# kevslinger/DTQN

Measured on AMD Instinct MI355X. Metric: env-steps/sec + TD-updates/sec, DiscreteCarFlag-v0 ctx=50 b=32, 1/2/4/8 GPU, higher is better.
Workload: dtype f32; 1 GPU; DiscreteCarFlag-v0 shapes (BASELINE config 1): ctx=50, d_model=64, 8 heads, 2 layers, obs 3 f32, 3 actions, batch 32 per GPU, history 50, device replay 2500 x 200 steps; global_batch=32, parallelism=dp1, sampler=device

## Files before the change

### dtqn_amd/_binding.py

```python
from __future__ import annotations

import ctypes
import os
import re
from typing import Dict, List, Tuple

REPO = os.path.dirname(os.path.dirname(os.path.abspath(__file__)))
HEADER = os.path.join(REPO, "include", "dtqn_hip.h")

_SCALARS = {
    "int32_t": ctypes.c_int32, "uint32_t": ctypes.c_uint32, "float": ctypes.c_float, "int": ctypes.c_int,
}


def _strip_comments(src: str) -> str:
    src = re.sub(r"/\*.*?\*/", "", src, flags=re.S)
    return re.sub(r"//[^\n]*", "", src)


def parse_structs(header_path: str = HEADER) -> Dict[str, List[Tuple[str, object]]]:
    src = _strip_comments(open(header_path).read())
    out: Dict[str, List[Tuple[str, object]]] = {}
    for m in re.finditer(r"typedef\s+struct\s+(\w+)\s*\{(.*?)\}\s*(\w+)\s*;", src, flags=re.S):
        name, body = m.group(3), m.group(2)
        fields: List[Tuple[str, object]] = []
        for decl in body.split(";"):
            decl = " ".join(decl.split())
            if not decl:
                continue
            if "*" in decl:
                for nm in decl.split("*")[-1].split(","):
                    fields.append((nm.strip(), ctypes.c_void_p))
                continue
            toks = decl.split(" ", 1)
            ctype = _SCALARS[toks[0]]
            for nm in toks[1].split(","):
                fields.append((nm.strip(), ctype))
        out[name] = fields
    return out


def parse_defines(header_path: str = HEADER) -> Dict[str, int]:
    src = _strip_comments(open(header_path).read())
    return {m.group(1): int(m.group(2)) for m in re.finditer(r"#define\s+(DTQN_\w+)\s+(-?\d+)\s*$", src, flags=re.M)}


def parse_functions(header_path: str = HEADER) -> List[str]:
    src = _strip_comments(open(header_path).read())
    src = re.sub(r"typedef\s+struct.*?\}\s*\w+\s*;", "", src, flags=re.S)
    return re.findall(r"\b(dtqn_\w+)\s*\(", src)


_STRUCTS = parse_structs()
DEFINES = parse_defines()
FUNCTIONS = sorted(set(parse_functions()))


def _make(name: str):
    return type(name, (ctypes.Structure,), {"_fields_": _STRUCTS[name]})


DtqnNet = _make("DtqnNet")
DtqnWJob = _make("DtqnWJob")
DtqnReplay = _make("DtqnReplay")
DtqnReplayRecord = _make("DtqnReplayRecord")
DtqnTd = _make("DtqnTd")


def load_library(path: str) -> ctypes.CDLL:
    lib = ctypes.CDLL(path)
    missing = [f for f in FUNCTIONS if not hasattr(lib, f)]
    if missing:
        raise OSError(f"{path} does not export {missing} (declared in include/dtqn_hip.h)")
    vp, i32, u32 = ctypes.c_void_p, ctypes.c_int, ctypes.c_uint32
    P = ctypes.POINTER
    protos = {
        "dtqn_net_init": [P(DtqnNet)],
        "dtqn_net_wjobs": [P(DtqnNet), P(DtqnWJob)],
        "dtqn_net_fill_frozen": [P(DtqnNet), vp],
        "dtqn_lds_bytes_forward": [P(DtqnNet), i32],
        "dtqn_lds_bytes_backward": [P(DtqnNet)],
        "dtqn_replay_apply": [P(DtqnReplay), vp, vp, i32, vp],
        "dtqn_replay_sample": [P(DtqnReplay), i32, i32, i32, i32, u32, vp, vp, vp, vp],
        "dtqn_replay_sample_at": [P(DtqnReplay), i32, i32, i32, i32, u32, i32, vp, vp, vp, vp],
        "dtqn_replay_push": [P(DtqnReplay), vp, vp, i32, vp],
        "dtqn_td_prefers_tiled": [P(DtqnNet), i32],
        "dtqn_net_tiled_twin": [P(DtqnNet), P(DtqnNet)],
        "dtqn_replay_gather_bag": [P(DtqnReplay), vp, vp, vp, i32, i32, u32, vp, vp, vp, vp],
        "dtqn_actor_forward": [P(DtqnNet), vp, vp, vp, i32, vp, vp, vp, i32, u32, u32, vp],
        "dtqn_actor_forward_batch": [P(DtqnNet), vp, vp, vp, i32, i32, vp, vp, vp, i32, u32, u32, vp],
        "dtqn_actor_greedy_batch": [P(DtqnNet), vp, vp, vp, i32, i32, vp, vp, vp, vp, i32, u32, u32, vp],
        "dtqn_debug_last_actor_live": [],
        "dtqn_forward_tiled_strided": [P(DtqnNet), vp, vp, vp, i32, i32, i32, vp, vp, vp],
        "dtqn_forward_bag": [P(DtqnNet), vp, vp, vp, vp, vp, i32, i32, vp, vp, i32, u32, u32, vp],
        "dtqn_forward": [P(DtqnNet), vp, vp, vp, i32, i32, vp, vp],
        "dtqn_forward_workspace_floats": [P(DtqnNet), i32],
        "dtqn_forward_tiled": [P(DtqnNet), vp, vp, vp, i32, i32, vp, vp, vp],
        "dtqn_td_row_split": [P(DtqnNet), i32],
        "dtqn_td_latency_mode": [P(DtqnNet), i32],
        "dtqn_td_wgrad_is_direct": [P(DtqnNet), i32],
        "dtqn_td_wgrad_splits": [P(DtqnNet), i32],
        "dtqn_td_wpack_floats": [P(DtqnNet)],
        "dtqn_td_wpack": [P(DtqnNet), P(DtqnTd), vp],
        "dtqn_td_wgrad_is_fused": [P(DtqnNet), P(DtqnTd)],
        "dtqn_td_norm_partials": [P(DtqnNet)],
        "dtqn_td_xch_floats": [P(DtqnNet), i32],
        "dtqn_td_xch_flags": [P(DtqnNet), i32],
        "dtqn_td_forward": [P(DtqnNet), P(DtqnReplay), P(DtqnTd), vp],
        "dtqn_td_forward_part": [P(DtqnNet), P(DtqnReplay), P(DtqnTd), i32, i32, i32, i32, vp],
        "dtqn_td_fwd_slices4_ok": [P(DtqnNet)],
        "dtqn_td_backward": [P(DtqnNet), P(DtqnReplay), P(DtqnTd), vp],
        "dtqn_td_backward_ahead": [P(DtqnNet), P(DtqnReplay), P(DtqnTd), P(DtqnTd), i32, vp],
        "dtqn_td_wgrad": [P(DtqnNet), P(DtqnTd), vp],
        "dtqn_td_reduce": [P(DtqnNet), P(DtqnTd), vp],
        "dtqn_td_gradnorm": [P(DtqnNet), P(DtqnTd), vp],
        "dtqn_td_clip_adam": [P(DtqnNet), P(DtqnTd), vp],
        "dtqn_img_prep_floats": [P(DtqnNet)],
        "dtqn_img_act_floats": [P(DtqnNet), i32],
        "dtqn_img_gact_floats": [P(DtqnNet), i32],
        "dtqn_img_wpart_floats": [P(DtqnNet)],
        "dtqn_img_prep": [P(DtqnNet), vp, vp, vp],
        "dtqn_img_encode": [P(DtqnNet), vp, vp, vp, vp, i32, vp, vp, vp, vp, vp, vp],
        "dtqn_img_backward": [P(DtqnNet), vp, vp, vp, vp, i32, vp, vp, vp, vp, vp, vp, vp],
        "dtqn_img_td_lists": [P(DtqnNet), P(DtqnReplay), P(DtqnTd), vp, vp, vp, vp, vp, vp, vp],
        "dtqn_forward_tiled_pre": [P(DtqnNet), vp, vp, vp, i32, i32, vp, vp, i32, u32, u32, vp],
        "dtqn_img_actor_stage_bytes": [P(DtqnNet), i32],
        "dtqn_img_actor_workspace_floats": [P(DtqnNet), i32],
        "dtqn_img_actor_forward_batch": [P(DtqnNet), vp, vp, i32, vp, vp, vp, i32, vp, vp, vp, i32, u32, u32, vp],
        "dtqn_img_actor_greedy_batch": [P(DtqnNet), vp, vp, i32, vp, vp, vp, i32, vp, vp, vp, vp, i32, u32, u32, vp],
        "dtqn_debug_last_img_actor_tokens": [],
        "dtqn_grad_workspace_floats": [P(DtqnNet), i32, i32],
        "dtqn_forward_train": [P(DtqnNet), vp, vp, vp, vp, vp, i32, i32, vp, vp, vp],
        "dtqn_backward_dq": [P(DtqnNet), vp, vp, vp, vp, vp, i32, i32, vp, vp, vp, vp, vp],
        "dtqn_forward_train_drop": [P(DtqnNet), vp, vp, vp, vp, vp, i32, i32, vp, vp, u32, i32, vp],
        "dtqn_backward_dq_drop": [P(DtqnNet), vp, vp, vp, vp, vp, i32, i32, vp, vp, vp, vp, u32, i32, vp],
        "dtqn_attn_weights": [P(DtqnNet), vp, i32, i32, vp, vp, vp],
        "dtqn_xch_publish": [vp, i32, vp],
        "dtqn_td_xreduce": [P(DtqnNet), P(DtqnTd), vp, vp, i32, i32, vp, vp, vp, vp],
        "dtqn_td_update": [P(DtqnNet), P(DtqnReplay), P(DtqnTd), vp],
        "dtqn_td_update_pipelined": [P(DtqnNet), P(DtqnReplay), P(DtqnTd), P(DtqnTd), i32, i32, vp],
        "dtqn_td_gradients_pipelined": [P(DtqnNet), P(DtqnReplay), P(DtqnTd), P(DtqnTd), i32, i32, vp],
        "dtqn_target_sync": [P(DtqnNet), vp, vp, vp],
        "dtqn_debug_set_profile_buffer": [vp],
        "dtqn_debug_last_packed_blocks": [],
        "dtqn_abi_version": [],
        "dtqn_build_info": [],
    }
    for name, argtypes in protos.items():
        fn = getattr(lib, name)
        fn.argtypes = argtypes
        fn.restype = ctypes.c_char_p if name == "dtqn_build_info" else (
            ctypes.c_longlong if name in ("dtqn_img_act_floats", "dtqn_img_gact_floats", "dtqn_img_wpart_floats",
                                                    "dtqn_grad_workspace_floats", "dtqn_img_actor_stage_bytes",
                                                    "dtqn_img_actor_workspace_floats") else ctypes.c_int)
    assert set(protos) == set(FUNCTIONS), sorted(set(protos) ^ set(FUNCTIONS))
    if lib.dtqn_abi_version() != DEFINES["DTQN_ABI_VERSION"]:
        raise OSError(f"{path}: ABI version {lib.dtqn_abi_version()} != header {DEFINES['DTQN_ABI_VERSION']}")
    return lib


GATES = {"res": DEFINES["DTQN_GATE_RES"], "gru": DEFINES["DTQN_GATE_GRU"]}
POS = {"learned": DEFINES["DTQN_POS_LEARNED"], "sin": DEFINES["DTQN_POS_SIN"], "none": DEFINES["DTQN_POS_NONE"]}


def make_net(lib, *, obs_dim, num_actions, embed_per_obs_dim=8, action_dim=0, inner_embed_size=64, num_heads=8,
             num_layers=2, history_len=50, gate="res", identity=False, pos="learned", discrete=False,
             vocab_sizes=0, dropout=0.0, bag_size=0, image=None) -> DtqnNet:
    net = DtqnNet()
    net.obs_dim, net.num_actions, net.embed_per_obs, net.action_dim = obs_dim, num_actions, embed_per_obs_dim, action_dim
    net.d_model, net.num_heads, net.num_layers, net.ctx_len = inner_embed_size, num_heads, num_layers, history_len
    if gate not in GATES:
        raise ValueError("Gate must be one of `gru`, `res`")
    net.gate, net.identity, net.pos = GATES[gate], int(bool(identity)), POS[str(pos)]
    net.discrete, net.vocab = int(bool(discrete)), int(vocab_sizes or 0)
    net.dropout = float(dropout)
    net.bag_size = int(bag_size)
    if image is not None:
        net.img_c, net.img_h, net.img_w = (int(v) for v in image)
        net.obs_dim = net.img_c * net.img_h * net.img_w
    rc = lib.dtqn_net_init(ctypes.byref(net))
    if rc != 0:
        raise NotImplementedError(
            f"dtqn_net_init rc={rc}: this DTQN variant/shape is outside the gfx950 kernels' coverage "
            f"(D={inner_embed_size}, H={num_heads}, L={history_len}, gate={gate}, dropout={dropout}, bag_size={bag_size}); see DESIGN.md")
    return net


def param_table(net: DtqnNet, width: int = 0) -> Dict[str, Tuple[int, Tuple[int, ...]]]:
    D, L, A, a = (width or net.d_model), net.ctx_len, net.num_actions, net.action_dim
    tab: Dict[str, Tuple[int, Tuple[int, ...]]] = {}
    if a > 0:
        tab["action_embedding.embedding.0.weight"] = (net.off_act_emb, (A, a))
    if net.img_c > 0:
        chans = [(net.img_c, 64), (64, 64), (64, 64), (64, 128), (128, 128)]
        offs = [(net.off_cw0, net.off_cb0), (net.off_cw1, net.off_cb1), (net.off_cw2, net.off_cb2), (net.off_cw3, net.off_cb3), (net.off_cw4, net.off_cb4)]
        for i, ((ci, co), (ow, ob)) in enumerate(zip(chans, offs)):
            tab[f"obs_embedding.observation_embedding.{2 * i}.weight"] = (ow, (co, ci, 3, 3))
            tab[f"obs_embedding.observation_embedding.{2 * i}.bias"] = (ob, (co,))
        tab["obs_embedding.observation_embedding.11.weight"] = (net.off_obs_w, (D - a, net.ke))
        tab["obs_embedding.observation_embedding.11.bias"] = (net.off_obs_b, (D - a,))
    elif net.discrete:
        tab["obs_embedding.observation_embedding.0.weight"] = (net.off_obs_tab, (net.vocab, net.embed_per_obs))
        tab["obs_embedding.observation_embedding.2.weight"] = (net.off_obs_w, (D - a, net.ke))
        tab["obs_embedding.observation_embedding.2.bias"] = (net.off_obs_b, (D - a,))
    else:
        tab["obs_embedding.observation_embedding.weight"] = (net.off_obs_w, (D - a, net.ke))
        tab["obs_embedding.observation_embedding.bias"] = (net.off_obs_b, (D - a,))
    tab["position_embedding.position_encoding"] = (net.off_pos, (1, L, D))
    gate_names = [("w_r.weight", net.go_w_r, (D, D)), ("u_r.weight", net.go_u_r, (D, D)),
                  ("w_z.weight", net.go_w_z, (D, D)), ("w_z.bias", net.go_b_z, (D,)),
                  ("u_z.weight", net.go_u_z, (D, D)), ("w_g.weight", net.go_w_g, (D, D)),
                  ("u_g.weight", net.go_u_g, (D, D))]
    for l in range(net.num_layers):
        base = net.off_layer0 + l * net.layer_stride
        pre = f"transformer_layers.{l}."
        tab[pre + "layernorm1.weight"] = (base + net.lo_ln1_w, (D,))
        tab[pre + "layernorm1.bias"] = (base + net.lo_ln1_b, (D,))
        tab[pre + "layernorm2.weight"] = (base + net.lo_ln2_w, (D,))
        tab[pre + "layernorm2.bias"] = (base + net.lo_ln2_b, (D,))
        tab[pre + "attention.in_proj_weight"] = (base + net.lo_in_w, (3 * D, D))
        tab[pre + "attention.in_proj_bias"] = (base + net.lo_in_b, (3 * D,))
        tab[pre + "attention.out_proj.weight"] = (base + net.lo_out_w, (D, D))
        tab[pre + "attention.out_proj.bias"] = (base + net.lo_out_b, (D,))
        tab[pre + "ffn.0.weight"] = (base + net.lo_f1_w, (4 * D, D))
        tab[pre + "ffn.0.bias"] = (base + net.lo_f1_b, (4 * D,))
        tab[pre + "ffn.2.weight"] = (base + net.lo_f2_w, (D, 4 * D))
        tab[pre + "ffn.2.bias"] = (base + net.lo_f2_b, (D,))
        if net.gate == GATES["gru"]:
            for gname, goff in (("attn_gate", net.off_gate_attn), ("mlp_gate", net.off_gate_mlp)):
                for nm, off, shp in gate_names:
                    tab[pre + f"{gname}.{nm}"] = (goff + off, shp)
    if net.bag_size > 0:
        tab["bag_attention.in_proj_weight"] = (net.off_bag_in_w, (3 * D, D))
        tab["bag_attention.in_proj_bias"] = (net.off_bag_in_b, (3 * D,))
        tab["bag_attention.out_proj.weight"] = (net.off_bag_out_w, (D, D))
        tab["bag_attention.out_proj.bias"] = (net.off_bag_out_b, (D,))
    tab["ffn.0.weight"] = (net.off_head1_w, (D, 2 * D if net.bag_size > 0 else D))
    tab["ffn.0.bias"] = (net.off_head1_b, (D,))
    tab["ffn.2.weight"] = (net.off_head2_w, (A, D))
    tab["ffn.2.bias"] = (net.off_head2_b, (A,))
    return tab


def ws_lite(net: DtqnNet) -> bool:
    return (not net.tiled) and net.d_model == 64 and (net.head_dim == 32 or (net.d_real > 0 and net.head_dim in (8, 16)))


def _grids(net: DtqnNet, key: str, real_shape, padded_shape):
    H, Hp = net.heads_real or net.num_heads, net.num_heads
    hd, hdp = net.hd_real or net.head_dim, net.head_dim
    if key.endswith("attention.in_proj_weight") or key.endswith("attention.in_proj_bias"):
        return (3, H, hd) + tuple(real_shape[1:]), (3, Hp, hdp) + tuple(padded_shape[1:])
    if key.endswith("attention.out_proj.weight"):
        return (real_shape[0], H, hd), (padded_shape[0], Hp, hdp)
    return tuple(real_shape), tuple(padded_shape)


def unpad_param(net: DtqnNet, key: str, padded, real_shape):
    if not net.d_real or tuple(padded.shape) == tuple(real_shape):
        return padded
    rg, pg = _grids(net, key, real_shape, padded.shape)
    return padded.reshape(pg)[tuple(slice(0, r) for r in rg)].reshape(tuple(real_shape))


def pad_param(net: DtqnNet, key: str, real, padded_shape):
    if not net.d_real or tuple(real.shape) == tuple(padded_shape):
        return real
    import numpy as _np
    out = _np.zeros(padded_shape, dtype=real.dtype) if isinstance(real, _np.ndarray) else real.new_zeros(tuple(padded_shape))
    rg, pg = _grids(net, key, real.shape, padded_shape)
    out.reshape(pg)[tuple(slice(0, r) for r in rg)] = real.reshape(rg)
    return out
```

### dtqn_amd/csrc/dtqn_api.cpp

```cpp
#include <hip/hip_runtime.h>

#include <cstdlib>

#include "dtqn_hip.h"
#include "dtqn_limits.h"

extern "C" const char* dtqn_build_info(void) {
#ifdef DTQN_BUILD_INFO
    return DTQN_BUILD_INFO;
#else
    return "dtqn_hip (unstamped build)";
#endif
}

static void* g_profile_buffer = nullptr;
extern "C" int dtqn_debug_set_profile_buffer(void* dev_buffer) {
    g_profile_buffer = dev_buffer;
    return DTQN_OK;
}
extern "C" void* dtqn_debug_profile_buffer(void) { return g_profile_buffer; }

static int policy_cus() {
    int dev = 0, n = 0;
    if (hipGetDevice(&dev) != hipSuccess || hipDeviceGetAttribute(&n, hipDeviceAttributeMultiprocessorCount, dev) != hipSuccess || n <= 0) return 256;
    return n;
}
extern "C" int dtqn_td_row_split(const DtqnNet* net, int batch) {
    if (!net || batch < 1) return 1;
    const int cus = policy_cus();
    const char* e = getenv("DTQN_ROW_SPLIT");
    if (e != nullptr && e[0] == '0') return 1;
    const bool covered = !net->tiled && net->lp == 64 && !net->identity &&
                         (net->d_model == 64 || (net->d_model == 128 && net->gate == DTQN_GATE_RES));
    if (!covered) return 1;
    if (e != nullptr && e[0] == '1') return 2;
    if (e != nullptr && e[0] == '4') return 4;
    if (3 * batch * 2 <= cus) return 4;
    if (net->d_model == 64) {
        if (batch * 4 <= cus) return 4;
        if (batch * 2 <= cus) return 2;
    }
    return 1;
}
extern "C" int dtqn_td_latency_mode(const DtqnNet* net, int batch) {
    if (dtqn_td_row_split(net, batch) < 2) return 0;
    const char* e = getenv("DTQN_ROW_SPLIT");
    if (e != nullptr && (e[0] == '1' || e[0] == '4')) return 1;
    return 3 * batch * 2 <= policy_cus() ? 1 : 0;
}
extern "C" int dtqn_td_prefers_tiled(const DtqnNet* net, int batch) {
    if (!net || batch < 1 || net->tiled) return 0;
    if (dtqn_ws_lite(net->tiled, net->d_model, net->head_dim, net->d_real))
        return dtqn_td_row_split(net, batch) == 4 && dtqn_td_latency_mode(net, batch) ? 0 : 1;
    const bool covered = net->d_model == 128 && net->gate == DTQN_GATE_RES && !net->identity && net->lp == 64 && net->dropout == 0.f &&
                         net->bag_size == 0;
    if (!covered) return 0;
    const char* e = getenv("DTQN_TRAIN_TILED");
    if (e != nullptr) return atoi(e) != 0 ? 1 : 0;
    return dtqn_td_row_split(net, batch) == 1 ? 1 : 0;
}
extern "C" int dtqn_td_xch_floats(const DtqnNet* net, int batch) {
    if (!net || batch < 1) return 0;
    return 3 * batch * net->num_layers * (3 * net->lp / 4) * 2 * net->d_model;
}
extern "C" int dtqn_td_xch_flags(const DtqnNet* net, int batch) {
    if (!net || batch < 1) return 0;
    return 3 * batch * net->num_layers * 6 + 16;
}

extern "C" int dtqn_td_update(const DtqnNet* net, const DtqnReplay* rp, const DtqnTd* td, void* stream) {
    int rc;
    if ((rc = dtqn_td_forward(net, rp, td, stream)) != DTQN_OK) return rc;
    if ((rc = dtqn_td_backward(net, rp, td, stream)) != DTQN_OK) return rc;
    if ((rc = dtqn_td_wgrad(net, td, stream)) != DTQN_OK) return rc;
    if ((rc = dtqn_td_reduce(net, td, stream)) != DTQN_OK) return rc;
    return dtqn_td_clip_adam(net, td, stream);
}

extern "C" int dtqn_td_gradients_pipelined(const DtqnNet* net, const DtqnReplay* rp, const DtqnTd* td, const DtqnTd* td_next, int have_target,
                                           int draw_step, void* stream) {
    int rc;
    if (draw_step < 0) return DTQN_ERR_ARG;
    if ((rc = dtqn_td_forward_part(net, rp, td, 0, 2, 4, draw_step, stream)) != DTQN_OK) return rc;
    if (!have_target && (rc = dtqn_td_forward_part(net, rp, td, 2, 1, 4, draw_step, stream)) != DTQN_OK) return rc;
    rc = td_next != nullptr ? dtqn_td_backward_ahead(net, rp, td, td_next, draw_step + 1, stream) : dtqn_td_backward(net, rp, td, stream);
    if (rc != DTQN_OK) return rc;
    if ((rc = dtqn_td_wgrad(net, td, stream)) != DTQN_OK) return rc;
    return dtqn_td_reduce(net, td, stream);
}
extern "C" int dtqn_td_update_pipelined(const DtqnNet* net, const DtqnReplay* rp, const DtqnTd* td, const DtqnTd* td_next, int have_target,
                                        int draw_step, void* stream) {
    const int rc = dtqn_td_gradients_pipelined(net, rp, td, td_next, have_target, draw_step, stream);
    return rc != DTQN_OK ? rc : dtqn_td_clip_adam(net, td, stream);
}

namespace dtqn {
int forward_infer(const DtqnNet* net, const float* theta, const float* obs, const uint8_t* actions, int batch, int n,
                  float* q_out, float* q_last_host, void* stream, float* xch, int32_t* xflags, const int32_t* last_rows, int in_rows,
                  uint32_t drop_seed, uint32_t drop_step, int train_mode);
int tiled_forward_actor(const DtqnNet* net, const float* theta, const float* obs, const uint8_t* actions, int batch, int n, int in_rows,
                        float* q_out, float* workspace, int train_mode, uint32_t drop_seed, uint32_t drop_step, hipStream_t stream, const int32_t* lens = nullptr);
int actor_compact(const DtqnNet* net, const void* ctx_host, void* ctx_dev, int n_envs, int n_max, hipStream_t stream);
int actor_greedy_rows(const int32_t* lens, const float* q, float* q_last, int32_t* action, int n_envs, int n_max, int A, hipStream_t stream);
void set_last_actor_live(int live);
}
extern "C" int dtqn_forward_tiled_strided(const DtqnNet* net, const float* theta, const float* obs, const uint8_t* actions,
                                          int batch, int n, int in_rows, float* q_out, float* workspace, void* stream);

extern "C" int dtqn_replay_push(const DtqnReplay* rp, const DtqnReplayRecord* recs_host, const float* obs_host, int n,
                                void* stream) {
    if (!rp || n < 0) return DTQN_ERR_ARG;
    if (n == 0) return DTQN_OK;
    if (!recs_host || !obs_host) return DTQN_ERR_ARG;
    return dtqn_replay_apply(rp, recs_host, obs_host, n, stream);
}

extern "C" int dtqn_actor_forward(const DtqnNet* net, const float* theta, const void* ctx_host, void* ctx_dev, int n,
                                  float* q_dev, float* q_last_host, float* workspace, int train_mode, uint32_t dropout_seed,
                                  uint32_t dropout_step, void* stream) {
    if (!net || !theta || !ctx_host || !ctx_dev || !q_dev || !q_last_host) return DTQN_ERR_ARG;
    if (n < 1 || n > net->ctx_len) return DTQN_ERR_ARG;
    hipStream_t s = (hipStream_t)stream;
    const size_t obs_bytes = sizeof(float) * (size_t)net->ctx_len * net->obs_dim;
    if (hipMemcpyAsync(ctx_dev, ctx_host, obs_bytes + (size_t)net->ctx_len, hipMemcpyHostToDevice, s) != hipSuccess) return DTQN_ERR_LAUNCH;
    const float* obs = static_cast<const float*>(ctx_dev);
    const uint8_t* actions = static_cast<const uint8_t*>(ctx_dev) + obs_bytes;
    if (!net->tiled) {
        const bool split = workspace != nullptr && n > net->lp / 2 && dtqn_td_row_split(net, 1) >= 2;
        float* xch = split ? workspace : nullptr;
        int32_t* xflags = split ? reinterpret_cast<int32_t*>(workspace + dtqn_td_xch_floats(net, 1)) : nullptr;
        return dtqn::forward_infer(net, theta, obs, actions, 1, n, q_dev, q_last_host, stream, xch, xflags, nullptr, 0, dropout_seed, dropout_step, train_mode);
    }
    const int rc = dtqn::tiled_forward_actor(net, theta, obs, actions, 1, n, n, q_dev, workspace, train_mode, dropout_seed, dropout_step, s);
    if (rc != DTQN_OK) return rc;
    if (hipMemcpyAsync(q_last_host, q_dev + (size_t)(n - 1) * net->num_actions, sizeof(float) * net->num_actions,
                       hipMemcpyDeviceToHost, s) != hipSuccess)
        return DTQN_ERR_LAUNCH;
    return DTQN_OK;
}

struct ActorBlock {
    const float* obs;
    const uint8_t* actions;
    const int32_t* lens;
};
static ActorBlock actor_block(const DtqnNet* net, void* base, int n_envs) {
    const size_t obs_bytes = sizeof(float) * (size_t)n_envs * net->ctx_len * net->obs_dim;
    const size_t act_bytes = (((size_t)n_envs * net->ctx_len) + 3) & ~(size_t)3;
    const uint8_t* p = static_cast<const uint8_t*>(base);
    return ActorBlock{static_cast<const float*>(base), p + obs_bytes, reinterpret_cast<const int32_t*>(p + obs_bytes + act_bytes)};
}
static int actor_batch_forward(const DtqnNet* net, const float* theta, const ActorBlock& b, int batch, int ws_envs, int n_max, float* q_dev,
                               float* q_last_host, float* workspace, int train_mode, uint32_t dropout_seed, uint32_t dropout_step,
                               void* stream) {
    const int L = net->ctx_len;
    if (net->tiled)
        return dtqn::tiled_forward_actor(net, theta, b.obs, b.actions, batch, n_max, L, q_dev, workspace, train_mode, dropout_seed,
                                         dropout_step, (hipStream_t)stream, b.lens);
    const bool split = workspace != nullptr && n_max > net->lp / 2 && dtqn_td_row_split(net, batch) >= 2;
    float* xch = split ? workspace : nullptr;
    int32_t* xflags = split ? reinterpret_cast<int32_t*>(workspace + dtqn_td_xch_floats(net, ws_envs)) : nullptr;
    return dtqn::forward_infer(net, theta, b.obs, b.actions, batch, n_max, q_dev, q_last_host, stream, xch, xflags, b.lens, L, dropout_seed,
                               dropout_step, train_mode);
}

extern "C" int dtqn_actor_forward_batch(const DtqnNet* net, const float* theta, const void* ctx_host, void* ctx_dev, int n_envs,
                                        int n_max, float* q_dev, float* q_last_host, float* workspace, int train_mode,
                                        uint32_t dropout_seed, uint32_t dropout_step, void* stream) {
    if (!net || !theta || !ctx_host || !ctx_dev || !q_dev || !q_last_host || n_envs < 1) return DTQN_ERR_ARG;
    if (n_max < 1 || n_max > net->ctx_len) return DTQN_ERR_ARG;
    hipStream_t s = (hipStream_t)stream;
    const int L = net->ctx_len;
    const size_t obs_bytes = sizeof(float) * (size_t)n_envs * L * net->obs_dim;
    const size_t act_bytes = (((size_t)n_envs * L) + 3) & ~(size_t)3;
    const size_t total = obs_bytes + act_bytes + sizeof(int32_t) * (size_t)n_envs;
    const int32_t* lens_h = reinterpret_cast<const int32_t*>(static_cast<const uint8_t*>(ctx_host) + obs_bytes + act_bytes);
    for (int i = 0; i < n_envs; ++i)
        if (lens_h[i] < 1 || lens_h[i] > n_max) return DTQN_ERR_ARG;
    if (hipMemcpyAsync(ctx_dev, ctx_host, total, hipMemcpyHostToDevice, s) != hipSuccess) return DTQN_ERR_LAUNCH;
    const ActorBlock b = actor_block(net, ctx_dev, n_envs);
    const int rc = actor_batch_forward(net, theta, b, n_envs, n_envs, n_max, q_dev, q_last_host, workspace, train_mode, dropout_seed,
                                       dropout_step, stream);
    if (rc != DTQN_OK || !net->tiled) return rc;
    for (int i = 0; i < n_envs; ++i)
        if (hipMemcpyAsync(q_last_host + (size_t)i * net->num_actions, q_dev + ((size_t)i * n_max + (lens_h[i] - 1)) * net->num_actions,
                           sizeof(float) * net->num_actions, hipMemcpyDeviceToHost, s) != hipSuccess)
            return DTQN_ERR_LAUNCH;
    return DTQN_OK;
}

extern "C" int dtqn_actor_greedy_batch(const DtqnNet* net, const float* theta, const void* ctx_host, void* ctx_dev, int n_envs,
                                       int n_max, float* q_dev, float* q_last_host, int32_t* action_host, float* workspace,
                                       int train_mode, uint32_t dropout_seed, uint32_t dropout_step, void* stream) {
    if (!net || !theta || !ctx_host || !ctx_dev || !q_dev || !q_last_host || !action_host || n_envs < 1) return DTQN_ERR_ARG;
    if (n_max < 0 || n_max > net->ctx_len) return DTQN_ERR_ARG;
    const ActorBlock h = actor_block(net, const_cast<void*>(ctx_host), n_envs);
    int live = 0;
    for (int i = 0; i < n_envs; ++i) {
        if (h.lens[i] < 0 || h.lens[i] > n_max) return DTQN_ERR_ARG;
        live += h.lens[i] > 0 ? 1 : 0;
    }
    dtqn::set_last_actor_live(live);
    if (live == 0) {
        for (int i = 0; i < n_envs; ++i) action_host[i] = -1;
        return DTQN_OK;
    }
    hipStream_t s = (hipStream_t)stream;
    int rc;
    if ((rc = dtqn::actor_compact(net, ctx_host, ctx_dev, n_envs, n_max, s)) != DTQN_OK) return rc;
    const ActorBlock b = actor_block(net, ctx_dev, n_envs);
    if ((rc = actor_batch_forward(net, theta, b, live, n_envs, n_max, q_dev, nullptr, workspace, train_mode, dropout_seed, dropout_step,
                                  stream)) != DTQN_OK)
        return rc;
    return dtqn::actor_greedy_rows(h.lens, q_dev, q_last_host, action_host, n_envs, n_max, net->num_actions, s);
}

extern "C" int dtqn_forward_train(const DtqnNet* net, const float* theta, const float* obs, const uint8_t* actions, const float* bag_obs,
                                  const uint8_t* bag_actions, int batch, int n, float* q_out, float* workspace, void* stream) {
    return dtqn_forward_train_drop(net, theta, obs, actions, bag_obs, bag_actions, batch, n, q_out, workspace, 0u, -1, stream);
}
extern "C" int dtqn_backward_dq(const DtqnNet* net, const float* theta, const float* obs, const uint8_t* actions, const float* bag_obs,
                                const uint8_t* bag_actions, int batch, int n, const float* dq, float* workspace, float* grad, float* dobs,
                                void* stream) {
    return dtqn_backward_dq_drop(net, theta, obs, actions, bag_obs, bag_actions, batch, n, dq, workspace, grad, dobs, 0u, -1, stream);
}
```

### dtqn_amd/csrc/dtqn_optim.hip

```cpp
#include <cstdlib>

#include "dtqn_device.hpp"

namespace dtqn {

constexpr int kOptThreads = 256;
constexpr int kOptVec = 4;
constexpr int kOptBlockElems = kOptThreads * kOptVec;

struct ReduceArgs {
    DtqnNet net;
    const float* gsplit;
    const float* small;
    const float* grd;
    float* grad;
    float* norm_partial;
    int32_t* step_counter;
    int batch, n_split;
    int n_parts;
};

__device__ __forceinline__ float block_sum(float v, float* red, int tid) {
    for (int m = 32; m >= 1; m >>= 1) v += __shfl_xor(v, m);
    if ((tid & 63) == 0) red[tid >> 6] = v;
    __syncthreads();
    float s = 0.f;
    for (int w = 0; w < kOptThreads / 64; ++w) s += red[w];
    __syncthreads();
    return s;
}

__global__ __launch_bounds__(kOptThreads) void dtqn_reduce_kernel(ReduceArgs a) {
    __shared__ float red[kOptThreads / 64];
    const DtqnNet& net = a.net;
    const int tid = (int)threadIdx.x;
    const int p0 = ((int)blockIdx.x * kOptThreads + tid) * kOptVec;
    if (blockIdx.x == 0 && tid == 0) a.step_counter[0] = a.step_counter[1];
    if (blockIdx.x == 0)
        for (int i = (int)gridDim.x + tid; i < a.n_parts; i += kOptThreads) a.norm_partial[i] = 0.f;
    float v[kOptVec] = {0.f, 0.f, 0.f, 0.f};
    if (p0 < net.n_trainable) {
        for (int s = 0; s < a.n_split; ++s) {
            const float4 x = ld4(a.gsplit + (size_t)s * net.n_trainable + p0);
            v[0] += x.x; v[1] += x.y; v[2] += x.z; v[3] += x.w;
        }
        st4(a.grad + p0, make_float4(v[0], v[1], v[2], v[3]));
    }
    const float ss = block_sum((v[0] * v[0] + v[1] * v[1]) + (v[2] * v[2] + v[3] * v[3]), red, tid);
    if (tid == 0) a.norm_partial[blockIdx.x] = ss;
}

struct NormArgs {
    const float* grad;
    float* norm_partial;
    int n, n_parts;
};
__global__ __launch_bounds__(kOptThreads) void dtqn_gradnorm_kernel(NormArgs a) {
    __shared__ float red[kOptThreads / 64];
    const int tid = (int)threadIdx.x;
    const int p0 = ((int)blockIdx.x * kOptThreads + tid) * kOptVec;
    if (blockIdx.x == 0)
        for (int i = (int)gridDim.x + tid; i < a.n_parts; i += kOptThreads) a.norm_partial[i] = 0.f;
    float ss = 0.f;
    if (p0 < a.n) {
        const float4 g = ld4(a.grad + p0);
        ss = (g.x * g.x + g.y * g.y) + (g.z * g.z + g.w * g.w);
    }
    ss = block_sum(ss, red, tid);
    if (tid == 0) a.norm_partial[blockIdx.x] = ss;
}

struct PublishArgs {
    int32_t* flag;
    int32_t gen;
};
__global__ void dtqn_xch_publish_kernel(PublishArgs a) {
    if (threadIdx.x == 0 && blockIdx.x == 0) DTQN_SYSTEM_STORE(a.flag, a.gen);
}
struct XreduceArgs {
    const float* const* peer_grad;
    int32_t* const* peer_flag;
    float* gsum;
    float* norm_partial;
    int32_t* status;
    int n, n_parts, world;
    int32_t gen;
    long long timeout_ticks;
    int32_t* own_flag;
};
__global__ __launch_bounds__(kOptThreads) void dtqn_xreduce_kernel(XreduceArgs a) {
    __shared__ float red[kOptThreads / 64];
    const int tid = (int)threadIdx.x;
    if (blockIdx.x == 0)
        for (int i = (int)gridDim.x + tid; i < a.n_parts; i += kOptThreads) a.norm_partial[i] = 0.f;
    if (a.own_flag != nullptr && blockIdx.x == 0 && tid == 0) DTQN_SYSTEM_STORE(a.own_flag, a.gen);
    if (tid < a.world) {
        const int32_t* f = a.peer_flag[tid];
        const long long t0 = wall_clock64();
        while ((int32_t)(DTQN_SYSTEM_LOAD(f) - a.gen) < 0) {
            if (wall_clock64() - t0 > a.timeout_ticks || DTQN_SYSTEM_LOAD(a.status) != 0) {
                DTQN_SYSTEM_STORE(a.status, (int32_t)1);
                break;
            }
            DTQN_SPIN_PAUSE();
        }
    }
    __syncthreads();
    const int p0 = ((int)blockIdx.x * kOptThreads + tid) * kOptVec;
    float v[kOptVec] = {0.f, 0.f, 0.f, 0.f};
    if (p0 < a.n) {
        for (int r = 0; r < a.world; ++r) {
            const int32_t* g = reinterpret_cast<const int32_t*>(a.peer_grad[r] + p0);
#pragma unroll
            for (int c = 0; c < kOptVec; ++c) v[c] += __int_as_float(DTQN_SYSTEM_LOAD(g + c));
        }
        st4(a.gsum + p0, make_float4(v[0], v[1], v[2], v[3]));
    }
    const float ss = block_sum((v[0] * v[0] + v[1] * v[1]) + (v[2] * v[2] + v[3] * v[3]), red, tid);
    if (tid == 0) a.norm_partial[blockIdx.x] = ss;
}

struct AdamArgs {
    float* theta;
    float* theta_tgt;
    const float* grad;
    float* m;
    float* v;
    const float* norm_partial;
    const float* stats_partial;
    float* stats;
    float* stats_ring;
    int32_t* step_counter;
    const int32_t* xstatus;
    int n, n_norm_parts, batch, history, tuf, ring_slots;
    int n_stat_parts;
    float lr, beta1, beta2, eps, clip, grad_scale;
};

__global__ __launch_bounds__(kOptThreads) void dtqn_clip_adam_kernel(AdamArgs a) {
    __shared__ float red[kOptThreads / 64];
    __shared__ double pw[2];
    const int tid = (int)threadIdx.x;
    const int p0 = ((int)blockIdx.x * kOptThreads + tid) * kOptVec;
    const bool mine = p0 < a.n;
    const float4 z4 = make_float4(0.f, 0.f, 0.f, 0.f);
    const float4 g4 = mine ? ld4(a.grad + p0) : z4;
    float4 m4 = mine ? ld4(a.m + p0) : z4, v4 = mine ? ld4(a.v + p0) : z4, p4 = mine ? ld4(a.theta + p0) : z4;
    float part = 0.f;
    for (int i = tid; i < a.n_norm_parts; i += kOptThreads) part += a.norm_partial[i];
    const float total = block_sum(part, red, tid);
    const float norm = sqrtf(total) * a.grad_scale;
    const int why = !isfinite(norm) ? 1 : (a.xstatus != nullptr && *a.xstatus != 0) ? 2 : (a.step_counter[3] != 0) ? 3 : 0;
    const bool finite = why == 0;
    const int k = a.step_counter[0] + 1;
    if (tid == 0 || tid == 64) {
        const double beta = tid == 0 ? (double)a.beta1 : (double)a.beta2;
        double r = 1.0, b = beta;
        for (unsigned e = (unsigned)k; e != 0u; e >>= 1) {
            if (e & 1u) r *= b;
            b *= b;
        }
        pw[tid >> 6] = 1.0 - r;
    }
    __syncthreads();
    const float bc1 = (float)pw[0], bc2_sqrt = (float)sqrt(pw[1]);
    const float coef = fminf(1.0f, a.clip / (norm + 1e-6f)) * a.grad_scale;
    const float step_size = a.lr / bc1;
    const bool sync_target = finite && a.tuf > 0 && (k % a.tuf) == 0;
    if (finite && mine) {
        const float g[4] = {g4.x * coef, g4.y * coef, g4.z * coef, g4.w * coef};
        float mm[4] = {m4.x, m4.y, m4.z, m4.w}, vv[4] = {v4.x, v4.y, v4.z, v4.w}, pp[4] = {p4.x, p4.y, p4.z, p4.w};
#pragma unroll
        for (int c = 0; c < 4; ++c) {
            mm[c] = mm[c] + (g[c] - mm[c]) * (1.0f - a.beta1);
            vv[c] = vv[c] * a.beta2 + (1.0f - a.beta2) * g[c] * g[c];
            const float denom = sqrtf(vv[c]) / bc2_sqrt + a.eps;
            pp[c] = pp[c] - step_size * (mm[c] / denom);
        }
        st4(a.m + p0, make_float4(mm[0], mm[1], mm[2], mm[3]));
        st4(a.v + p0, make_float4(vv[0], vv[1], vv[2], vv[3]));
        const float4 pn = make_float4(pp[0], pp[1], pp[2], pp[3]);
        st4(a.theta + p0, pn);
        if (sync_target) st4(a.theta_tgt + p0, pn);
    }
    if (blockIdx.x == gridDim.x - 1) {
        float se = 0.f, sq = 0.f, sy = 0.f, mxq = -INFINITY, mnq = INFINITY, mxy = -INFINITY, mny = INFINITY;
        const int call_prev = a.step_counter[2];
        for (int b = tid; b < a.n_stat_parts; b += kOptThreads) {
            const float* sp = a.stats_partial + (size_t)b * 8;
            se += sp[0]; sq += sp[1]; mxq = fmaxf(mxq, sp[2]); mnq = fminf(mnq, sp[3]);
            sy += sp[4]; mxy = fmaxf(mxy, sp[5]); mny = fminf(mny, sp[6]);
        }
        se = block_sum(se, red, tid); sq = block_sum(sq, red, tid); sy = block_sum(sy, red, tid);
        for (int mk = 32; mk >= 1; mk >>= 1) {
            mxq = fmaxf(mxq, __shfl_xor(mxq, mk)); mnq = fminf(mnq, __shfl_xor(mnq, mk));
            mxy = fmaxf(mxy, __shfl_xor(mxy, mk)); mny = fminf(mny, __shfl_xor(mny, mk));
        }
        __shared__ float mm4[4][kOptThreads / 64];
        if ((tid & 63) == 0) { mm4[0][tid >> 6] = mxq; mm4[1][tid >> 6] = mnq; mm4[2][tid >> 6] = mxy; mm4[3][tid >> 6] = mny; }
        __syncthreads();
        if (tid == 0) {
            for (int w = 1; w < kOptThreads / 64; ++w) {
                mxq = fmaxf(mxq, mm4[0][w]); mnq = fminf(mnq, mm4[1][w]); mxy = fmaxf(mxy, mm4[2][w]); mny = fminf(mny, mm4[3][w]);
            }
            const float cnt = (float)a.batch * (float)a.history;
            a.stats[0] = se / cnt;
            a.stats[1] = norm;
            a.stats[2] = mxq; a.stats[3] = sq / cnt; a.stats[4] = mnq;
            a.stats[5] = mxy; a.stats[6] = sy / cnt; a.stats[7] = mny;
            a.stats[8] = fminf(1.0f, a.clip / (norm + 1e-6f));
            a.stats[9] = (float)k;
            a.stats[10] = sync_target ? 1.f : 0.f;
            a.stats[11] = (float)why;
            if (finite) a.step_counter[1] = k;
            else a.step_counter[3] = 1;
            const int call = call_prev + 1;
            a.step_counter[2] = call;
            if (a.stats_ring != nullptr) {
                unsigned long long* slot = reinterpret_cast<unsigned long long*>(a.stats_ring) + (size_t)((call - 1) % a.ring_slots) * 12;
                const unsigned long long tag = (unsigned long long)__float_as_uint((float)(call & 0x7fffff)) << 32;
                const float vals[12] = {se / cnt, norm, mxq, sq / cnt, mnq, mxy, sy / cnt, mny, fminf(1.0f, a.clip / (norm + 1e-6f)), (float)k,
                                        sync_target ? 1.f : 0.f, (float)why};
                for (int i = 0; i < 12; ++i) DTQN_SYSTEM_STORE(slot + i, tag | (unsigned long long)__float_as_uint(vals[i]));
            }
        }
    }
}

struct CopyArgs {
    const float* src;
    float* dst;
    int n;
};
__global__ __launch_bounds__(kOptThreads) void dtqn_copy_kernel(CopyArgs a) {
    const int p0 = ((int)blockIdx.x * kOptThreads + (int)threadIdx.x) * kOptVec;
    if (p0 < a.n) st4(a.dst + p0, ld4(a.src + p0));
}

}

using namespace dtqn;

static int opt_blocks(int n) { return (n + kOptBlockElems - 1) / kOptBlockElems; }

extern "C" int dtqn_td_reduce(const DtqnNet* net, const DtqnTd* td, void* stream) {
    if (!net || !td) return DTQN_ERR_ARG;
    if (td->n_norm_blocks != opt_blocks(net->n_trainable)) return DTQN_ERR_ARG;
    if (dtqn_td_wgrad_is_direct(net, td->batch)) return DTQN_OK;
    ReduceArgs a;
    a.net = *net;
    a.gsplit = td->gsplit; a.small = td->small; a.grd = td->grd; a.grad = td->grad;
    a.norm_partial = td->norm_partial; a.step_counter = td->step_counter;
    a.batch = td->batch; a.n_split = td->n_split; a.n_parts = dtqn_td_norm_partials(net);
    (void)hipGetLastError();
    hipLaunchKernelGGL(dtqn_reduce_kernel, dim3(td->n_norm_blocks), dim3(kOptThreads), 0, (hipStream_t)stream, a);
    return hipGetLastError() == hipSuccess ? DTQN_OK : DTQN_ERR_LAUNCH;
}

extern "C" int dtqn_td_gradnorm(const DtqnNet* net, const DtqnTd* td, void* stream) {
    if (!net || !td) return DTQN_ERR_ARG;
    if (td->n_norm_blocks != opt_blocks(net->n_trainable)) return DTQN_ERR_ARG;
    NormArgs a;
    a.grad = td->grad; a.norm_partial = td->norm_partial; a.n = net->n_trainable; a.n_parts = dtqn_td_norm_partials(net);
    (void)hipGetLastError();
    hipLaunchKernelGGL(dtqn_gradnorm_kernel, dim3(td->n_norm_blocks), dim3(kOptThreads), 0, (hipStream_t)stream, a);
    return hipGetLastError() == hipSuccess ? DTQN_OK : DTQN_ERR_LAUNCH;
}

extern "C" int dtqn_xch_publish(int32_t* own_flag_dev, int32_t gen, void* stream) {
    if (!own_flag_dev) return DTQN_ERR_ARG;
    PublishArgs a;
    a.flag = own_flag_dev; a.gen = gen;
    (void)hipGetLastError();
    hipLaunchKernelGGL(dtqn_xch_publish_kernel, dim3(1), dim3(64), 0, (hipStream_t)stream, a);
    return hipGetLastError() == hipSuccess ? DTQN_OK : DTQN_ERR_LAUNCH;
}

extern "C" int dtqn_td_xreduce(const DtqnNet* net, const DtqnTd* td, const void* peer_grad_ptrs_dev, const void* peer_flag_ptrs_dev, int world,
                               int32_t gen, float* gsum_dev, int32_t* status_dev, int32_t* own_flag_dev, void* stream) {
    if (!net || !td || !peer_grad_ptrs_dev || !peer_flag_ptrs_dev || !gsum_dev || !status_dev) return DTQN_ERR_ARG;
    if (world < 1 || world > kOptThreads) return DTQN_ERR_ARG;
    if (td->n_norm_blocks != opt_blocks(net->n_trainable)) return DTQN_ERR_ARG;
    XreduceArgs a;
    a.peer_grad = static_cast<const float* const*>(peer_grad_ptrs_dev);
    a.peer_flag = static_cast<int32_t* const*>(peer_flag_ptrs_dev);
    a.gsum = gsum_dev; a.norm_partial = td->norm_partial; a.status = status_dev;
    a.n = net->n_trainable; a.n_parts = dtqn_td_norm_partials(net); a.world = world; a.gen = gen; a.own_flag = own_flag_dev;
    const char* tmo = getenv("DTQN_XCH_TIMEOUT_MS");
    const long long ms = td->xch_timeout_ms > 0 ? (long long)td->xch_timeout_ms : tmo != nullptr && atoll(tmo) > 0 ? atoll(tmo) : 5000ll;
    a.timeout_ticks = ms * 100000ll;
    (void)hipGetLastError();
    hipLaunchKernelGGL(dtqn_xreduce_kernel, dim3(td->n_norm_blocks), dim3(kOptThreads), 0, (hipStream_t)stream, a);
    return hipGetLastError() == hipSuccess ? DTQN_OK : DTQN_ERR_LAUNCH;
}

extern "C" int dtqn_td_clip_adam(const DtqnNet* net, const DtqnTd* td, void* stream) {
    if (!net || !td) return DTQN_ERR_ARG;
    if (td->n_norm_blocks != opt_blocks(net->n_trainable)) return DTQN_ERR_ARG;
    AdamArgs a;
    a.theta = td->theta_pol; a.theta_tgt = td->theta_tgt; a.grad = td->grad; a.m = td->adam_m; a.v = td->adam_v;
    a.norm_partial = td->norm_partial; a.stats_partial = td->stats_partial; a.stats = td->stats;
    a.step_counter = td->step_counter;
    a.xstatus = td->xstatus;
    a.stats_ring = td->stats_ring; a.ring_slots = td->stats_ring_slots > 0 ? td->stats_ring_slots : 1;
    a.n = net->n_trainable; a.n_norm_parts = dtqn_td_norm_partials(net); a.batch = td->batch; a.history = td->history;
    a.n_stat_parts = td->batch * (td->row_split > 1 ? td->row_split : 1);
    a.tuf = td->target_update_frequency;
    a.lr = td->lr; a.beta1 = td->beta1; a.beta2 = td->beta2; a.eps = td->eps; a.clip = td->grad_norm_clip;
    a.grad_scale = td->grad_scale;
    (void)hipGetLastError();
    hipLaunchKernelGGL(dtqn_clip_adam_kernel, dim3(td->n_norm_blocks + 1), dim3(kOptThreads), 0, (hipStream_t)stream, a);
    return hipGetLastError() == hipSuccess ? DTQN_OK : DTQN_ERR_LAUNCH;
}

extern "C" int dtqn_target_sync(const DtqnNet* net, const float* theta_pol, float* theta_tgt, void* stream) {
    if (!net || !theta_pol || !theta_tgt) return DTQN_ERR_ARG;
    CopyArgs a;
    a.src = theta_pol; a.dst = theta_tgt; a.n = net->n_theta;
    (void)hipGetLastError();
    hipLaunchKernelGGL(dtqn_copy_kernel, dim3(opt_blocks(net->n_theta)), dim3(kOptThreads), 0, (hipStream_t)stream, a);
    return hipGetLastError() == hipSuccess ? DTQN_OK : DTQN_ERR_LAUNCH;
}
```

### dtqn_amd/csrc/dtqn_wgrad.hip

```cpp
#include <mutex>
#include "dtqn_device.hpp"
#include "dtqn_wgrad_direct.hpp"

namespace dtqn {

constexpr int kMaxWJobs = 48;
struct WgradArgs {
    DtqnNet net;
    DtqnWJob jobs[kMaxWJobs];
    const float* act;
    const float* grd;
    float* gsplit;
    const float* small;
    int batch, n_split, n_jobs;
    int n_small;
    int row_split;
    int small_blocks;
    int xcd_map;
    int n_wtiles;
};

__device__ __forceinline__ void small_partials_block(const WgradArgs& a, int sb, int split) {
    const DtqnNet& net = a.net;
    const int D = net.d_model;
    const int n_ln = net.num_layers * 4 * D;
    const int n_tab = net.discrete ? net.vocab * net.embed_per_obs : 0;
    const int n_act = net.action_dim > 0 ? net.num_actions * net.action_dim : 0;
    const int b_lo = (int)((long long)a.batch * split / a.n_split);
    const int b_hi = (int)((long long)a.batch * (split + 1) / a.n_split);
    float* out = a.gsplit + (size_t)split * net.n_trainable;
    for (int e = sb * 1024 + (int)threadIdx.x; e < min(a.n_small, (sb + 1) * 1024); e += DTQN_THREADS) {
        int dst, src;
        const float* base = a.small;
        size_t stride = (size_t)net.sp_stride;
        if (e < n_ln) {
            const int l = e / (4 * D);
            dst = net.off_layer0 + l * net.layer_stride + (e - l * 4 * D);
            src = net.so_ln + e;
        } else if (e < n_ln + n_tab) {
            dst = net.off_obs_tab + (e - n_ln);
            src = net.so_tab + (e - n_ln);
        } else if (e < n_ln + n_tab + n_act) {
            dst = net.off_act_emb + (e - n_ln - n_tab);
            src = net.so_act + (e - n_ln - n_tab);
        } else {
            dst = net.off_pos + (e - n_ln - n_tab - n_act);
            src = net.go_dx0 + (e - n_ln - n_tab - n_act);
            base = a.grd;
            stride = (size_t)net.grd_stride;
        }
        float v = 0.f;
        const int per = base == a.small ? a.row_split * net.sp_parts : 1;
        for (int b = b_lo * per; b < b_hi * per; ++b) v += base[(size_t)b * stride + src];
        out[dst] = v;
    }
}

__global__ __launch_bounds__(DTQN_THREADS, 2) void dtqn_wgrad_kernel(WgradArgs a) {
    const Thr t = make_thr();
    const DtqnNet& net = a.net;
    const int LP = net.lp;
    const int P = a.n_wtiles * a.n_split, per = (P + 7) / 8, tile_blocks = per * 8, id = (int)blockIdx.x;
    if (id >= tile_blocks) {
        small_partials_block(a, (id - tile_blocks) % a.small_blocks, (id - tile_blocks) / a.small_blocks);
        return;
    }
    const int pair = a.xcd_map ? (id % 8) * per + id / 8 : id;
    if (pair >= P) return;
    const int split = pair / a.n_wtiles, tile = pair - split * a.n_wtiles;
    int j = 0;
    for (int k = 1; k < a.n_jobs; ++k)
        if (a.jobs[k].tile0 <= tile) j = k;
    const DtqnWJob& job = a.jobs[j];
    const int local = tile - job.tile0;
    const int bn = local / job.tiles_k, bk = local - bn * job.tiles_k;
    const int nbase = bn * 64, kbase = bk * 64;
    const float* xbase = (job.x_in_act ? a.act : a.grd) + job.x_off;
    const size_t xstride = job.x_in_act ? (size_t)net.act_stride : (size_t)net.grd_stride;
    const float* ybase = a.grd + job.dy_off;
    const size_t ystride = (size_t)net.grd_stride;
    const int ycol = nbase + 4 * t.i, xcol = kbase + 4 * t.i;
    const bool yok = ycol < job.ldy, xok = xcol < job.ldx;

    f32x4 acc[4][4];
#pragma unroll
    for (int cn = 0; cn < 4; ++cn)
#pragma unroll
        for (int ck = 0; ck < 4; ++ck) acc[cn][ck] = zero4();
    float4 bsum = make_float4(0.f, 0.f, 0.f, 0.f);

    const int b_lo = (int)((long long)a.batch * split / a.n_split);
    const int b_hi = (int)((long long)a.batch * (split + 1) / a.n_split);
    const bool fast = LP % 16 == 0;
    const int NSUB = fast ? LP / 16 : 4;
    const int steps_per_sub = fast ? 4 : (LP / 4 + NSUB - 1) / NSUB;
    const int units = (b_hi - b_lo) * NSUB * job.n_layers;
    const float4 z4 = make_float4(0.f, 0.f, 0.f, 0.f);
    auto unit_ptrs = [&](int u, const float*& yp, const float*& xp, int& s_lo, int& s_hi) {
        const int lyr = u / ((b_hi - b_lo) * NSUB), ul = u - lyr * (b_hi - b_lo) * NSUB;
        const int b = b_lo + ul / NSUB, sub = ul - (ul / NSUB) * NSUB;
        s_lo = sub * steps_per_sub;
        s_hi = min(LP / 4, s_lo + steps_per_sub);
        yp = ybase + (size_t)b * ystride + (size_t)lyr * job.dy_lstride + (size_t)t.kq * job.ldy + ycol;
        xp = xbase + (size_t)b * xstride + (size_t)lyr * job.x_lstride + (size_t)t.kq * job.ldx + xcol;
    };
    if (fast) {
        float4 av[3][4], bv[3][4];
        auto unit_load = [&](int u, float4 (&a4)[4], float4 (&b4)[4]) {
            const float *yp, *xp;
            int s_lo, s_hi;
            unit_ptrs(u, yp, xp, s_lo, s_hi);
#pragma unroll
            for (int k = 0; k < 4; ++k) {
                a4[k] = yok ? ld4(yp + (size_t)4 * (s_lo + k) * job.ldy) : z4;
                b4[k] = xok ? ld4(xp + (size_t)4 * (s_lo + k) * job.ldx) : z4;
            }
        };
        auto unit_mma = [&](const float4 (&a4)[4], const float4 (&b4)[4]) {
#pragma unroll
            for (int k = 0; k < 4; ++k) {
                bsum.x += a4[k].x; bsum.y += a4[k].y; bsum.z += a4[k].z; bsum.w += a4[k].w;
                const float aa[4] = {a4[k].x, a4[k].y, a4[k].z, a4[k].w};
                const float bb[4] = {b4[k].x, b4[k].y, b4[k].z, b4[k].w};
#pragma unroll
                for (int cn = 0; cn < 4; ++cn)
#pragma unroll
                    for (int ck = 0; ck < 4; ++ck) acc[cn][ck] = mfma16(aa[cn], bb[ck], acc[cn][ck]);
            }
        };
        constexpr int W = DTQN_WAVES;
        int u = t.wave;
        if (u < units) unit_load(u, av[0], bv[0]);
        if (LP <= 64) {
            for (; u < units; u += 2 * W) {
                if (u + W < units) unit_load(u + W, av[1], bv[1]);
                unit_mma(av[0], bv[0]);
                if (u + W < units) {
                    if (u + 2 * W < units) unit_load(u + 2 * W, av[0], bv[0]);
                    unit_mma(av[1], bv[1]);
                }
            }
        } else {
            if (u + W < units) unit_load(u + W, av[1], bv[1]);
            for (; u < units; u += 3 * W) {
                if (u + 2 * W < units) unit_load(u + 2 * W, av[2], bv[2]);
                unit_mma(av[0], bv[0]);
                if (u + W < units) {
                    if (u + 3 * W < units) unit_load(u + 3 * W, av[0], bv[0]);
                    unit_mma(av[1], bv[1]);
                    if (u + 2 * W < units) {
                        if (u + 4 * W < units) unit_load(u + 4 * W, av[1], bv[1]);
                        unit_mma(av[2], bv[2]);
                    }
                }
            }
        }
    }
    for (int u = fast ? units : t.wave; u < units; u += DTQN_WAVES) {
        const float *yp, *xp;
        int s_lo, s_hi;
        unit_ptrs(u, yp, xp, s_lo, s_hi);
        float4 av = (yok && s_lo < s_hi) ? ld4(yp + (size_t)4 * s_lo * job.ldy) : z4;
        float4 bv = (xok && s_lo < s_hi) ? ld4(xp + (size_t)4 * s_lo * job.ldx) : z4;
#pragma unroll 2
        for (int s = s_lo; s < s_hi; ++s) {
            const float4 an = (yok && s + 1 < s_hi) ? ld4(yp + (size_t)4 * (s + 1) * job.ldy) : z4;
            const float4 bn = (xok && s + 1 < s_hi) ? ld4(xp + (size_t)4 * (s + 1) * job.ldx) : z4;
            bsum.x += av.x; bsum.y += av.y; bsum.z += av.z; bsum.w += av.w;
            const float aa[4] = {av.x, av.y, av.z, av.w};
            const float bb[4] = {bv.x, bv.y, bv.z, bv.w};
#pragma unroll
            for (int cn = 0; cn < 4; ++cn)
#pragma unroll
                for (int ck = 0; ck < 4; ++ck) acc[cn][ck] = mfma16(aa[cn], bb[ck], acc[cn][ck]);
            av = an;
            bv = bn;
        }
    }
    bsum.x += __shfl_xor(bsum.x, 16); bsum.y += __shfl_xor(bsum.y, 16); bsum.z += __shfl_xor(bsum.z, 16); bsum.w += __shfl_xor(bsum.w, 16);
    bsum.x += __shfl_xor(bsum.x, 32); bsum.y += __shfl_xor(bsum.y, 32); bsum.z += __shfl_xor(bsum.z, 32); bsum.w += __shfl_xor(bsum.w, 32);

    constexpr int SLD = 68;
    float* slab = reinterpret_cast<float*>(dtqn_smem) + (size_t)t.wave * 65 * SLD;
#pragma unroll
    for (int cn = 0; cn < 4; ++cn)
#pragma unroll
        for (int r = 0; r < 4; ++r)
            st4(slab + (4 * (t.kq * 4 + r) + cn) * SLD + 4 * t.i,
                make_float4(acc[cn][0][r], acc[cn][1][r], acc[cn][2][r], acc[cn][3][r]));
    if (t.kq == 0) st4(slab + 64 * SLD + 4 * t.i, bsum);
    __syncthreads();
    const float* s0 = reinterpret_cast<const float*>(dtqn_smem);
    float* out = a.gsplit + (size_t)split * net.n_trainable;
    for (int idx = t.tid; idx < 64 * 16; idx += DTQN_THREADS) {
        const int nl = idx >> 4, k4 = (idx & 15) * 4;
        const int n = nbase + nl, k = kbase + k4;
        if (n < job.N && k < job.K) {
            float4 v = ld4(s0 + nl * SLD + k4);
#pragma unroll
            for (int wv = 1; wv < DTQN_WAVES; ++wv) {
                const float4 x = ld4(s0 + (size_t)wv * 65 * SLD + nl * SLD + k4);
                v.x += x.x; v.y += x.y; v.z += x.z; v.w += x.w;
            }
            float* op = out + job.w_off + (size_t)n * job.K + k;
            if (k + 3 < job.K && (job.K & 3) == 0) {
                st4(op, v);
            } else {
                const float vv[4] = {v.x, v.y, v.z, v.w};
                for (int c = 0; c < 4; ++c)
                    if (k + c < job.K) op[c] = vv[c];
            }
        }
    }
    if (job.b_off >= 0 && bk == 0 && t.tid < 64) {
        const int n = nbase + t.tid;
        if (n < job.N) {
            float v = 0.f;
#pragma unroll
            for (int wv = 0; wv < DTQN_WAVES; ++wv) v += s0[(size_t)wv * 65 * SLD + 64 * SLD + t.tid];
            out[job.b_off + n] = v;
        }
    }
}

constexpr int kLdsTK = 32, kLdsLDY = 128, kLdsLDX = 160, kLdsThreads = 512;
struct WgradLdsJob {
    DtqnWJob j;
    int tile0;
};
struct WgradLdsArgs {
    DtqnNet net;
    WgradLdsJob jobs[kMaxWJobs];
    const float* act;
    const float* grd;
    float* gsplit;
    int batch, n_split, n_jobs, n_tiles;
};
__global__ __launch_bounds__(kLdsThreads, 2) void dtqn_wgrad_lds_kernel(WgradLdsArgs a) {
    const Thr t = make_thr();
    const DtqnNet& net = a.net;
    const int LP = net.lp;
    float* Ys = reinterpret_cast<float*>(dtqn_smem);
    float* Xs = Ys + kLdsTK * kLdsLDY;
    const int pair = (int)blockIdx.x, split = pair / a.n_tiles, tile = pair - split * a.n_tiles;
    int jx = 0;
    for (int k = 1; k < a.n_jobs; ++k)
        if (a.jobs[k].tile0 <= tile) jx = k;
    const DtqnWJob& job = a.jobs[jx].j;
    const int local = tile - a.jobs[jx].tile0, tk = job.K / 128;
    const int bn = local / tk, bk = local - bn * tk, nbase = bn * 128, kbase = bk * 128;
    const float* xbase = (job.x_in_act ? a.act : a.grd) + job.x_off + kbase;
    const size_t xstride = job.x_in_act ? (size_t)net.act_stride : (size_t)net.grd_stride;
    const float* ybase = a.grd + job.dy_off + nbase;
    const size_t ystride = (size_t)net.grd_stride;
    const int b_lo = (int)((long long)a.batch * split / a.n_split), b_hi = (int)((long long)a.batch * (split + 1) / a.n_split);
    const int live_rows = net.bag_size > 0 ? LP : net.ctx_len;
    const int cps = (live_rows + kLdsTK - 1) / kLdsTK, nb = b_hi - b_lo, nchunks = job.n_layers * nb * cps;
    f32x4 acc[4][2];
#pragma unroll
    for (int cn = 0; cn < 4; ++cn) { acc[cn][0] = zero4(); acc[cn][1] = zero4(); }
    float bsum = 0.f;
    const bool want_bias = job.b_off >= 0 && bk == 0;
    const int sr = t.tid >> 5, sc = (t.tid & 31) * 4;
    float4 yr[2], xr[2];
    auto chunk_load = [&](int c) {
        const int lyr = c / (nb * cps), rem = c - lyr * nb * cps, b = rem / cps, r0 = (rem - b * cps) * kLdsTK;
        const float* yp = ybase + (size_t)(b_lo + b) * ystride + (size_t)lyr * job.dy_lstride + (size_t)r0 * job.ldy + sc;
        const float* xp = xbase + (size_t)(b_lo + b) * xstride + (size_t)lyr * job.x_lstride + (size_t)r0 * job.ldx + sc;
#pragma unroll
        for (int k = 0; k < 2; ++k) {
            yr[k] = ld4(yp + (size_t)(sr + 16 * k) * job.ldy);
            xr[k] = ld4(xp + (size_t)(sr + 16 * k) * job.ldx);
        }
    };
    const int wn = t.wave >> 2, wk = t.wave & 3;
    const float* ya = Ys + t.kq * kLdsLDY + 64 * wn + 4 * t.i;
    const float* xa = Xs + t.kq * kLdsLDX + 32 * wk + 2 * t.i;
    if (nchunks > 0) chunk_load(0);
    for (int c = 0; c < nchunks; ++c) {
        __syncthreads();
#pragma unroll
        for (int k = 0; k < 2; ++k) {
            st4(Ys + (sr + 16 * k) * kLdsLDY + sc, yr[k]);
            st4(Xs + (sr + 16 * k) * kLdsLDX + sc, xr[k]);
        }
        __syncthreads();
        if (c + 1 < nchunks) chunk_load(c + 1);
        const int r0c = (c % cps) * kLdsTK, smax = live_rows - r0c >= kLdsTK ? kLdsTK / 4 : (live_rows - r0c + 3) / 4;
#pragma unroll
        for (int s = 0; s < kLdsTK / 4; ++s) {
            if (s >= smax) break;
            const float4 a4 = ld4(ya + 4 * s * kLdsLDY);
            const float2 b2 = *reinterpret_cast<const float2*>(xa + 4 * s * kLdsLDX);
            const float aa[4] = {a4.x, a4.y, a4.z, a4.w};
#pragma unroll
            for (int cn = 0; cn < 4; ++cn) {
                acc[cn][0] = mfma16(aa[cn], b2.x, acc[cn][0]);
                acc[cn][1] = mfma16(aa[cn], b2.y, acc[cn][1]);
            }
        }
        if (want_bias && t.tid < 128) {
#pragma unroll 8
            for (int r = 0; r < kLdsTK; ++r) bsum += Ys[r * kLdsLDY + t.tid];
        }
    }
    float* out = a.gsplit + (size_t)split * net.n_trainable;
#pragma unroll
    for (int cn = 0; cn < 4; ++cn)
#pragma unroll
        for (int r = 0; r < 4; ++r) {
            const int n = nbase + 64 * wn + 4 * (4 * t.kq + r) + cn, k = kbase + 32 * wk + 2 * t.i;
            *reinterpret_cast<float2*>(out + job.w_off + (size_t)n * job.K + k) = make_float2(acc[cn][0][r], acc[cn][1][r]);
        }
    if (want_bias && t.tid < 128) out[job.b_off + nbase + t.tid] = bsum;
}
static inline bool wgrad_lds_job(const DtqnNet& net, const DtqnWJob& j) {
    return net.tiled && j.N % 128 == 0 && j.K % 128 == 0 && j.ldy % 4 == 0 && j.ldx % 4 == 0;
}
static inline bool wgrad_lds_enabled(const DtqnNet& net) {
    const char* e = getenv("DTQN_WGRAD_LDS");
    return net.tiled && net.d_model % 128 == 0 && net.img_c <= 0 && !(e != nullptr && atoi(e) == 0);
}

struct WgradDirectArgs {
    DtqnNet net;
    DtqnWJob jobs[kMaxWJobs];
    int dtile0[kMaxWJobs];
    const float* act;
    const float* grd;
    float* grad;
    const float* small;
    float* norm_partial;
    int32_t* step_counter;
    int batch, n_jobs, n_small, row_split;
    int n_tiles, n_parts;
    int slots;
    int xcd_tile0[8], xcd_ntiles[8];
    int xcd_map;
    int small_per;
};

__global__ __launch_bounds__(kDirectThreads) void dtqn_wgrad_direct_kernel(WgradDirectArgs a) {
    const Thr t = make_thr();
    const DtqnNet& net = a.net;
    const int tid = t.tid;
    float* red = reinterpret_cast<float*>(dtqn_smem);
    float* slabs = red + kDirectWaves;
    float ss = 0.f;
    const int b = (int)blockIdx.x, tile_blocks = a.slots * 8;
    if (b == 0 && tid == 0) a.step_counter[0] = a.step_counter[1];
    if (b == 0)
        for (int i = (int)gridDim.x + tid; i < a.n_parts; i += kDirectThreads) a.norm_partial[i] = 0.f;
    const int tile = b >= tile_blocks ? a.n_tiles : !a.xcd_map ? b : b / 8 < a.xcd_ntiles[b % 8] ? a.xcd_tile0[b % 8] + b / 8 : a.n_tiles;
    const DirectCtx ctx{a.act, a.grd, a.small, a.grad, a.batch, a.row_split, a.n_small};
    if (b >= tile_blocks) {
        ss = a.small_per == 2 * kDSmall ? direct_small<false, 2 * kDSmall, kDirectWaves>(net, ctx, b - tile_blocks, slabs, t)
                                        : direct_small<false, kDSmall, kDirectWaves>(net, ctx, b - tile_blocks, slabs, t);
    } else if (tile < a.n_tiles) {
        int j = 0;
        for (int k = 1; k < a.n_jobs; ++k)
            if (a.dtile0[k] <= tile) j = k;
        ss = direct_tile<false, kDirectWaves>(net, ctx, a.jobs[j], tile - a.dtile0[j], slabs, t);
    }
    direct_norm_partial<kDirectWaves>(ss, red, a.norm_partial, b, t);
}

static int direct_tiles(const DtqnNet* net, const DtqnWJob* jobs, int* dtile0) {
    int tiles = 0;
    for (int j = 0; j < net->n_wjobs; ++j) {
        if (dtile0) dtile0[j] = tiles;
        tiles += direct_tiles_of(jobs[j]);
    }
    return tiles;
}
struct DirectPlan {
    int dtile0[kMaxWJobs];
    int n_tiles, slots, grid;
    int small_per;
    int grid_max;
    int xcd_tile0[8], xcd_ntiles[8];
};
static DirectPlan direct_plan(const DtqnNet* net, const DtqnWJob* jobs) {
    DirectPlan p;
    p.n_tiles = direct_tiles(net, jobs, p.dtile0);
    const int per = (p.n_tiles + 7) / 8;
    for (int x = 0; x < 8; ++x) {
        p.xcd_tile0[x] = x * per < p.n_tiles ? x * per : p.n_tiles;
        p.xcd_ntiles[x] = p.n_tiles - p.xcd_tile0[x] < per ? p.n_tiles - p.xcd_tile0[x] : per;
    }
    p.slots = per;
    static_assert(2 * kDSmall / 64 <= kDirectWaves && (size_t)(2 * kDSmall / 64) * kDirectWaves * 64 <= kDirectLdsFloats - kDirectWaves, "small-partial block fits");
    const int n_small = small_elems(net), g1 = p.slots * 8 + (n_small + kDSmall - 1) / kDSmall, g2 = p.slots * 8 + (n_small + 2 * kDSmall - 1) / (2 * kDSmall);
    const int cus = fuse_cu_count();
    p.small_per = (cus > 0 && g1 > cus && g2 <= cus) ? 2 * kDSmall : kDSmall;
    const char* e = getenv("DTQN_DSMALL");
    if (e != nullptr && (atoi(e) == kDSmall || atoi(e) == 2 * kDSmall)) p.small_per = atoi(e);
    p.grid = p.small_per == kDSmall ? g1 : g2;
    p.grid_max = g1;
    return p;
}

}

using namespace dtqn;

extern "C" int dtqn_td_wgrad_splits(const DtqnNet* net, int batch) {
    if (!net || batch < 1) return 1;
    int n = batch < 16 ? batch : 16;
    if (net->n_wjobs <= kMaxWJobs && wgrad_lds_enabled(*net)) {
        DtqnWJob jobs[kMaxWJobs];
        if (dtqn_net_wjobs(net, jobs) == DTQN_OK) {
            int tiles = 0;
            for (int j = 0; j < net->n_wjobs; ++j)
                if (wgrad_lds_job(*net, jobs[j])) tiles += (jobs[j].N / 128) * (jobs[j].K / 128);
            if (tiles > 0) {
                const int cus = device_cu_count() > 0 ? device_cu_count() : 256;
                const char* e = getenv("DTQN_WGRAD_SLOTS");
                const int per_cu = e != nullptr && atoi(e) > 0 ? atoi(e) : 2;
                n = per_cu * cus / tiles;
                n = n < 1 ? 1 : (n > batch ? batch : n);
                n = n > 64 ? 64 : n;
            }
        }
    }
    return n;
}

extern "C" int dtqn_td_wgrad_is_direct(const DtqnNet* net, int batch) {
    if (!net || batch < 1 || net->n_wjobs > kMaxWJobs) return 0;
    if (net->img_c > 0) return 0;
    const char* e = getenv("DTQN_WGRAD_DIRECT");
    if (e != nullptr) return atoi(e) != 0 ? 1 : 0;
    const int gru_layers = net->gate == DTQN_GATE_GRU ? net->num_layers : 1, bag_sets = net->bag_size > 0 ? 2 : 1;
    const int layers = gru_layers > bag_sets ? gru_layers : bag_sets;
    return (long long)batch * net->lp * layers <= kDirectMaxTokens ? 1 : 0;
}

extern "C" int dtqn_td_norm_partials(const DtqnNet* net) {
    if (!net || net->n_wjobs > kMaxWJobs) return 0;
    DtqnWJob jobs[kMaxWJobs];
    if (dtqn_net_wjobs(net, jobs) != DTQN_OK) return 0;
    const int opt = (net->n_trainable + 1023) / 1024, dir = direct_plan(net, jobs).grid_max;
    return opt > dir ? opt : dir;
}

static int wgrad_direct(const DtqnNet* net, const DtqnTd* td, hipStream_t stream) {
    WgradDirectArgs a;
    a.net = *net;
    if (dtqn_net_wjobs(net, a.jobs) != DTQN_OK) return DTQN_ERR_CONFIG;
    for (int j = 0; j < net->n_wjobs; ++j)
        if ((long long)td->batch * net->lp * a.jobs[j].n_layers > kDirectMaxTokens) return DTQN_ERR_CONFIG;
    const DirectPlan plan = direct_plan(net, a.jobs);
    a.n_tiles = plan.n_tiles; a.slots = plan.slots; a.small_per = plan.small_per;
    for (int j = 0; j < net->n_wjobs; ++j) a.dtile0[j] = plan.dtile0[j];
    for (int x = 0; x < 8; ++x) { a.xcd_tile0[x] = plan.xcd_tile0[x]; a.xcd_ntiles[x] = plan.xcd_ntiles[x]; }
    a.act = td->act; a.grd = td->grd; a.grad = td->grad; a.small = td->small;
    a.norm_partial = td->norm_partial; a.step_counter = td->step_counter;
    a.batch = td->batch; a.n_jobs = net->n_wjobs; a.n_small = small_elems(net);
    a.row_split = td->row_split > 1 ? td->row_split : 1;
    a.n_parts = dtqn_td_norm_partials(net);
    const char* xm = getenv("DTQN_WGRAD_XCD");
    a.xcd_map = xm != nullptr ? atoi(xm) : 1;
    const int grid = plan.grid;
    const size_t lds = kDirectLdsFloats * sizeof(float);
    (void)hipGetLastError();
    hipLaunchKernelGGL(dtqn_wgrad_direct_kernel, dim3(grid), dim3(kDirectThreads), lds, stream, a);
    return hipGetLastError() == hipSuccess ? DTQN_OK : DTQN_ERR_LAUNCH;
}

struct WgradLane {
    hipStream_t s;
    hipEvent_t fork, join;
    int state;
};
static WgradLane* wgrad_lane() {
    static WgradLane lanes[kMaxDevices] = {};
    const char* e = getenv("DTQN_WGRAD_SIDE");
    if (e != nullptr && atoi(e) == 0) return nullptr;
    int dev = 0;
    if (hipGetDevice(&dev) != hipSuccess || dev < 0 || dev >= kMaxDevices) return nullptr;
    WgradLane& l = lanes[dev];
    if (l.state == 0) {
        l.state = (hipStreamCreateWithFlags(&l.s, hipStreamNonBlocking) == hipSuccess &&
                   hipEventCreateWithFlags(&l.fork, hipEventDisableTiming) == hipSuccess &&
                   hipEventCreateWithFlags(&l.join, hipEventDisableTiming) == hipSuccess) ? 1 : -1;
        (void)hipGetLastError();
    }
    return l.state == 1 ? &l : nullptr;
}

extern "C" int dtqn_td_wgrad(const DtqnNet* net, const DtqnTd* td, void* stream) {
    if (!net || !td || td->batch < 1 || td->n_split < 1) return DTQN_ERR_ARG;
    if (net->n_wjobs > kMaxWJobs) return DTQN_ERR_CONFIG;
    if (dtqn_td_wgrad_is_fused(net, td)) return DTQN_OK;
    if (dtqn_td_wgrad_is_direct(net, td->batch)) return wgrad_direct(net, td, (hipStream_t)stream);
    WgradArgs a;
    a.net = *net;
    if (dtqn_net_wjobs(net, a.jobs) != DTQN_OK) return DTQN_ERR_CONFIG;
    a.n_jobs = net->n_wjobs;
    a.n_wtiles = net->n_wtiles;
    WgradLdsArgs la;
    bool have_lds = false;
    if (wgrad_lds_enabled(*net)) {
        la.net = *net;
        la.n_jobs = 0; la.n_tiles = 0;
        int keep = 0, tiles = 0;
        for (int j = 0; j < net->n_wjobs; ++j) {
            if (wgrad_lds_job(*net, a.jobs[j])) {
                la.jobs[la.n_jobs].j = a.jobs[j];
                la.jobs[la.n_jobs].tile0 = la.n_tiles;
                la.n_tiles += (a.jobs[j].N / 128) * (a.jobs[j].K / 128);
                ++la.n_jobs;
            } else {
                a.jobs[keep] = a.jobs[j];
                a.jobs[keep].tile0 = tiles;
                tiles += a.jobs[keep].tiles_n * a.jobs[keep].tiles_k;
                ++keep;
            }
        }
        if (la.n_jobs > 0) {
            a.n_jobs = keep; a.n_wtiles = tiles;
            la.act = td->act; la.grd = td->grd; la.gsplit = td->gsplit; la.batch = td->batch; la.n_split = td->n_split;
            have_lds = true;
        }
    }
    WgradLane* lane = have_lds ? wgrad_lane() : nullptr;
    static std::mutex lane_mu;
    std::unique_lock<std::mutex> lk(lane_mu, std::defer_lock);
    hipStream_t small_stream = (hipStream_t)stream;
    if (lane != nullptr) {
        lk.lock();
        if (hipEventRecord(lane->fork, (hipStream_t)stream) == hipSuccess && hipStreamWaitEvent(lane->s, lane->fork, 0) == hipSuccess) small_stream = lane->s;
        else { lane = nullptr; (void)hipGetLastError(); }
    }
    a.act = td->act; a.grd = td->grd; a.gsplit = td->gsplit; a.small = td->small;
    a.batch = td->batch; a.n_split = td->n_split;
    a.row_split = td->row_split > 1 ? td->row_split : 1;
    a.n_small = net->num_layers * 4 * net->d_model + (net->discrete ? net->vocab * net->embed_per_obs : 0) +
                (net->action_dim > 0 ? net->num_actions * net->action_dim : 0) +
                (net->pos == DTQN_POS_LEARNED ? net->ctx_len * net->d_model : 0);
    const int small_blocks = (a.n_small + 1023) / 1024;
    a.small_blocks = small_blocks;
    const char* xm = getenv("DTQN_WGRAD_XCD");
    a.xcd_map = xm != nullptr ? atoi(xm) : 1;
    const int tile_blocks = (a.n_wtiles * td->n_split + 7) / 8 * 8;
    const size_t lds = (size_t)DTQN_WAVES * 65 * 68 * sizeof(float);
    static size_t attr_lds[kMaxDevices] = {};
    raise_lds_limit(reinterpret_cast<const void*>(&dtqn_wgrad_kernel), lds, attr_lds);
    (void)hipGetLastError();
    hipLaunchKernelGGL(dtqn_wgrad_kernel, dim3(tile_blocks + small_blocks * td->n_split), dim3(DTQN_THREADS), lds, small_stream, a);
    if (hipGetLastError() != hipSuccess) return DTQN_ERR_LAUNCH;
    if (lane != nullptr && hipEventRecord(lane->join, lane->s) != hipSuccess) return DTQN_ERR_LAUNCH;
    if (have_lds) {
        const size_t llds = (size_t)kLdsTK * (kLdsLDY + kLdsLDX) * sizeof(float);
        (void)hipGetLastError();
        hipLaunchKernelGGL(dtqn_wgrad_lds_kernel, dim3(la.n_tiles * td->n_split), dim3(kLdsThreads), llds, (hipStream_t)stream, la);
        if (hipGetLastError() != hipSuccess) return DTQN_ERR_LAUNCH;
    }
    if (lane != nullptr && hipStreamWaitEvent((hipStream_t)stream, lane->join, 0) != hipSuccess) return DTQN_ERR_LAUNCH;
    return DTQN_OK;
}
```

### dtqn_amd/csrc/dtqn_wgrad_direct.hpp

```cpp
#pragma once
#include "dtqn_device.hpp"

namespace dtqn {

#ifndef DTQN_DIRECT_WAVES
#define DTQN_DIRECT_WAVES 16
#endif
constexpr int kDirectWaves = DTQN_DIRECT_WAVES;
constexpr int kFuseWaves = 8;
constexpr int kDirectThreads = kDirectWaves * 64;
constexpr int kDirectMaxTokens = 2048;
constexpr int kDTN = 16, kDTK = 32;
constexpr int kDGroup = 8;
#ifndef DTQN_DSMALL
#define DTQN_DSMALL 128
#endif
constexpr int kDSmall = DTQN_DSMALL;
constexpr int kDSmallFused = 256;
constexpr size_t direct_lds_floats(int waves) { return waves + (size_t)waves * (kDTN + 1) * (kDTK + 4); }
constexpr size_t kDirectLdsFloats = direct_lds_floats(kDirectWaves);

struct DirectCtx {
    const float* act;
    const float* grd;
    const float* small;
    float* grad;
    int batch, row_split, n_small;
};

template <bool SC1>
__device__ __forceinline__ float direct_ld(const float* base, const DtqnRsrc& rs, size_t idx) {
    if constexpr (SC1) return dtqn_xch_load1(rs, (int)(idx * 4));
    else return base[idx];
}

template <bool SC1, int WV>
__device__ __forceinline__ float direct_tile(const DtqnNet& net, const DirectCtx& a, const DtqnWJob& job, int local, float* slabs, const Thr& t) {
    const int LP = net.lp, tid = t.tid;
    float ss = 0.f;
    const int tiles_k = (job.K + kDTK - 1) / kDTK;
    const int tiles_n = (job.N + kDTN - 1) / kDTN;
    const bool k_major = tiles_k > tiles_n;
    const int bn = k_major ? local % tiles_n : local / tiles_k, bk = k_major ? local / tiles_n : local - bn * tiles_k;
    const int nbase = bn * kDTN, kbase = bk * kDTK;
    const float* xbase = (job.x_in_act ? a.act : a.grd) + job.x_off;
    const size_t xstride = job.x_in_act ? (size_t)net.act_stride : (size_t)net.grd_stride;
    const size_t ystride = (size_t)net.grd_stride;
    const DtqnRsrc grs = DTQN_XCH_RSRC(a.grd, (size_t)a.batch * net.grd_stride * 4);
    const int ycol = nbase + t.i, xcol = kbase + 2 * t.i;
    const bool yok = ycol < job.ldy, xok = xcol < job.ldx;
    f32x4 acc[2] = {zero4(), zero4()};
    float bsum = 0.f;
    const int nsub = LP / 16;
    const int per_layer = a.batch * nsub, units = per_layer * job.n_layers;
    const int mine = (units - t.wave + WV - 1) / WV;
    constexpr int kMaxGroups = (kDirectMaxTokens / 16 + WV * kDGroup - 1) / (WV * kDGroup);
    constexpr int NBUF = kMaxGroups > 1 ? 2 : 1;
    float av[NBUF][kDGroup][4];
    float2 bv[NBUF][kDGroup][4];
    const int ycol_c = yok ? ycol : 0, xcol_c = xok ? xcol : 0;
    const int wv = __builtin_amdgcn_readfirstlane(t.wave);
    int u_lyr = 0, u_sq = wv / nsub, u_sub = wv - u_sq * nsub, u_m = 0;
    while (u_sq >= a.batch) { u_sq -= a.batch; ++u_lyr; }
    const int inc_sq = WV / nsub, inc_sub = WV - inc_sq * nsub;
    const size_t ylane = (size_t)job.dy_off + (size_t)t.kq * job.ldy + ycol_c;
    const float* xlane = xbase + (size_t)t.kq * job.ldx + xcol_c;
    auto group_load = [&](float (&a4)[kDGroup][4], float2 (&b4)[kDGroup][4]) {
#pragma unroll
        for (int q = 0; q < kDGroup; ++q) {
            const bool live = u_m < mine;
            const int lyr = live ? u_lyr : 0, sq = live ? u_sq : 0, sub = live ? u_sub : 0;
            const size_t yp = ylane + (size_t)sq * ystride + (size_t)lyr * job.dy_lstride + (size_t)(sub * 16) * job.ldy;
            const float* xp = xlane + (size_t)sq * xstride + (size_t)lyr * job.x_lstride + (size_t)(sub * 16) * job.ldx;
#pragma unroll
            for (int k = 0; k < 4; ++k) {
                a4[q][k] = direct_ld<SC1>(a.grd, grs, yp + (size_t)4 * k * job.ldy);
                b4[q][k] = *reinterpret_cast<const float2*>(xp + (size_t)4 * k * job.ldx);
            }
            ++u_m;
            u_sub += inc_sub; u_sq += inc_sq;
            if (u_sub >= nsub) { u_sub -= nsub; ++u_sq; }
            while (u_sq >= a.batch) { u_sq -= a.batch; ++u_lyr; }
        }
    };
    auto group_mma = [&](int g, const float (&a4)[kDGroup][4], const float2 (&b4)[kDGroup][4]) {
#pragma unroll
        for (int q = 0; q < kDGroup; ++q) {
            const float keep = (yok && g * kDGroup + q < mine) ? 1.f : 0.f;
#pragma unroll
            for (int k = 0; k < 4; ++k) {
                const float av_ = keep != 0.f ? a4[q][k] : 0.f;
                bsum += av_;
                acc[0] = mfma16(av_, b4[q][k].x, acc[0]);
                acc[1] = mfma16(av_, b4[q][k].y, acc[1]);
            }
        }
    };
    const int ngroups = (mine + kDGroup - 1) / kDGroup;
    if constexpr (kMaxGroups == 1) {
        group_load(av[0], bv[0]);
        DTQN_SCHED_FENCE();
        group_mma(0, av[0], bv[0]);
    } else {
        constexpr int B1 = NBUF - 1;
        if (ngroups > 0) group_load(av[0], bv[0]);
        DTQN_SCHED_FENCE();
        int g = 0;
        for (; g + 2 < ngroups; g += 2) {
            group_load(av[B1], bv[B1]);
            DTQN_SCHED_FENCE();
            group_mma(g, av[0], bv[0]);
            DTQN_SCHED_FENCE();
            group_load(av[0], bv[0]);
            DTQN_SCHED_FENCE();
            group_mma(g + 1, av[B1], bv[B1]);
            DTQN_SCHED_FENCE();
        }
        if (g + 1 < ngroups) {
            group_load(av[B1], bv[B1]);
            DTQN_SCHED_FENCE();
            group_mma(g, av[0], bv[0]);
            DTQN_SCHED_FENCE();
            group_mma(g + 1, av[B1], bv[B1]);
        } else if (g < ngroups) {
            group_mma(g, av[0], bv[0]);
        }
    }
    bsum += __shfl_xor(bsum, 16);
    bsum += __shfl_xor(bsum, 32);
    constexpr int SLD = kDTK + 4;
    float* slab = slabs + (size_t)t.wave * (kDTN + 1) * SLD;
#pragma unroll
    for (int r = 0; r < 4; ++r)
        *reinterpret_cast<float2*>(slab + (t.kq * 4 + r) * SLD + 2 * t.i) = make_float2(acc[0][r], acc[1][r]);
    if (t.kq == 0) slab[kDTN * SLD + t.i] = bsum;
    __syncthreads();
    if (tid < kDTN * (kDTK / 4)) {
        const int nl = tid / (kDTK / 4), k4 = (tid % (kDTK / 4)) * 4;
        const int n = nbase + nl, k = kbase + k4;
        if (n < job.N && k < job.K) {
            float4 v = ld4(slabs + nl * SLD + k4);
#pragma unroll
            for (int w = 1; w < WV; ++w) {
                const float4 x = ld4(slabs + (size_t)w * (kDTN + 1) * SLD + nl * SLD + k4);
                v.x += x.x; v.y += x.y; v.z += x.z; v.w += x.w;
            }
            float* op = a.grad + job.w_off + (size_t)n * job.K + k;
            if (k + 3 < job.K && (job.K & 3) == 0) {
                st4(op, v);
                ss = (v.x * v.x + v.y * v.y) + (v.z * v.z + v.w * v.w);
            } else {
                const float vv[4] = {v.x, v.y, v.z, v.w};
                for (int c = 0; c < 4; ++c)
                    if (k + c < job.K) { op[c] = vv[c]; ss += vv[c] * vv[c]; }
            }
        }
    } else if (tid >= 256 && tid < 256 + kDTN && job.b_off >= 0 && bk == 0) {
        const int nl = tid - 256, n = nbase + nl;
        if (n < job.N) {
            float v = 0.f;
#pragma unroll
            for (int w = 0; w < WV; ++w) v += slabs[(size_t)w * (kDTN + 1) * SLD + kDTN * SLD + nl];
            a.grad[job.b_off + n] = v;
            ss = v * v;
        }
    }
    return ss;
}

template <bool SC1, int PER, int WV>
__device__ __forceinline__ float direct_small(const DtqnNet& net, const DirectCtx& a, int sb, float* slabs, const Thr& t) {
    constexpr int HN = PER / 64;
    static_assert(HN <= WV, "one finishing wave per 64 elements");
    const int D = net.d_model;
    const int n_ln = net.num_layers * 4 * D;
    const int n_tab = net.discrete ? net.vocab * net.embed_per_obs : 0;
    const int n_act = net.action_dim > 0 ? net.num_actions * net.action_dim : 0;
    const DtqnRsrc grs = DTQN_XCH_RSRC(a.grd, (size_t)a.batch * net.grd_stride * 4);
    const DtqnRsrc srs = DTQN_XCH_RSRC(a.small, (size_t)a.batch * a.row_split * net.sp_parts * net.sp_stride * 4);
    float ss = 0.f;
    int dst[HN];
#pragma unroll
    for (int h = 0; h < HN; ++h) {
        dst[h] = -1;
        const int e = sb * PER + h * 64 + t.lane;
        float v = 0.f;
        if (e < a.n_small) {
            int src;
            bool in_small = true;
            size_t stride = (size_t)net.sp_stride;
            if (e < n_ln) {
                const int l = e / (4 * D);
                dst[h] = net.off_layer0 + l * net.layer_stride + (e - l * 4 * D);
                src = net.so_ln + e;
            } else if (e < n_ln + n_tab) {
                dst[h] = net.off_obs_tab + (e - n_ln);
                src = net.so_tab + (e - n_ln);
            } else if (e < n_ln + n_tab + n_act) {
                dst[h] = net.off_act_emb + (e - n_ln - n_tab);
                src = net.so_act + (e - n_ln - n_tab);
            } else {
                dst[h] = net.off_pos + (e - n_ln - n_tab - n_act);
                src = net.go_dx0 + (e - n_ln - n_tab - n_act);
                in_small = false;
                stride = (size_t)net.grd_stride;
            }
            const int cnt = a.batch * (in_small ? a.row_split * net.sp_parts : 1);
#pragma unroll 8
            for (int q = t.wave; q < cnt; q += WV)
                v += in_small ? direct_ld<SC1>(a.small, srs, (size_t)q * stride + src) : direct_ld<SC1>(a.grd, grs, (size_t)q * stride + src);
        }
        slabs[(h * WV + t.wave) * 64 + t.lane] = v;
    }
    __syncthreads();
    if (t.wave < HN) {
        int d = -1;
#pragma unroll
        for (int h = 0; h < HN; ++h) d = t.wave == h ? dst[h] : d;
        if (d >= 0) {
            float tot = 0.f;
#pragma unroll
            for (int w = 0; w < WV; ++w) tot += slabs[(t.wave * WV + w) * 64 + t.lane];
            a.grad[d] = tot;
            ss = tot * tot;
        }
    }
    return ss;
}

template <int WV>
__device__ __forceinline__ void direct_norm_partial(float ss, float* red, float* norm_partial, int slot, const Thr& t) {
    ss = wave_sum(ss);
    __syncthreads();
    if (t.lane == 0) red[t.wave] = ss;
    __syncthreads();
    if (t.tid == 0) {
        float tot = 0.f;
        for (int w = 0; w < WV; ++w) tot += red[w];
        norm_partial[slot] = tot;
    }
}

inline int direct_tiles_of(const DtqnWJob& j) { return ((j.N + kDTN - 1) / kDTN) * ((j.K + kDTK - 1) / kDTK); }
inline int small_elems(const DtqnNet* net) {
    return net->num_layers * 4 * net->d_model + (net->discrete ? net->vocab * net->embed_per_obs : 0) +
           (net->action_dim > 0 ? net->num_actions * net->action_dim : 0) +
           (net->pos == DTQN_POS_LEARNED ? net->ctx_len * net->d_model : 0);
}

constexpr int kFuseMaxJobs = 16;
constexpr int kFuseMaxEvents = 12;
constexpr int kFuseDeparted = kFuseMaxEvents;
constexpr int kFuseWords = 16;
struct FuseArgs {
    int n_role;
    int n_chain;
    int n_jobs, n_tiles, n_items, n_small, n_parts;
    DtqnWJob jobs[kFuseMaxJobs];
    int dtile0[kFuseMaxJobs];
    int job_event[kFuseMaxJobs];
    float* grad;
    float* norm_partial;
    int32_t* step_counter;
    int32_t* counters;
};

__device__ __forceinline__ void fuse_wait(int32_t* counter, int target, const Thr& t) {
    if (t.tid == 0)
        while (DTQN_AGENT_LOAD(counter) < target) DTQN_SPIN_PAUSE_LONG();
    __syncthreads();
}

template <int NW>
__device__ __forceinline__ void fuse_role(const DtqnNet& net, const FuseArgs& f, const DirectCtx& ctx, int w, float* smem, const Thr& t) {
    static_assert(NW == kFuseWaves, "the weight-gradient workgroups of the backward launch have its eight waves");
    float* red = smem;
    float* slabs = smem + NW;
    float ss = 0.f;
    if (w == 0 && t.tid == 0) f.step_counter[0] = f.step_counter[1];
    if (w == 0)
        for (int i = f.n_role + t.tid; i < f.n_parts; i += NW * 64) f.norm_partial[i] = 0.f;
    const int per_xcd = f.n_role / 8, slot = (w % 8) * per_xcd + w / 8;
    int waited = -1;
#ifndef DTQN_FUSE_DEBUG_PLAINLD
#define DTQN_FUSE_DEBUG_PLAINLD 0
#endif
#ifdef DTQN_FUSE_DEBUG_NOROLE
    for (int p = f.n_items; p < f.n_items; p += f.n_role) {
#else
    for (int p = slot; p < f.n_items; p += f.n_role) {
#endif
        __syncthreads();
        if (p < f.n_tiles) {
            int j = 0;
            for (int k = 1; k < f.n_jobs; ++k)
                if (f.dtile0[k] <= p) j = k;
            const int ev = f.job_event[j];
            if (ev > waited) { fuse_wait(f.counters + ev, f.n_chain, t); waited = ev; }
            ss += direct_tile<!DTQN_FUSE_DEBUG_PLAINLD, NW>(net, ctx, f.jobs[j], p - f.dtile0[j], slabs, t);
        } else {
            if (net.num_layers > waited) { fuse_wait(f.counters + net.num_layers, f.n_chain, t); waited = net.num_layers; }
            ss += direct_small<!DTQN_FUSE_DEBUG_PLAINLD, kDSmallFused, NW>(net, ctx, p - f.n_tiles, slabs, t);
        }
    }
    direct_norm_partial<NW>(ss, red, f.norm_partial, w, t);
    if (net.num_layers > waited) fuse_wait(f.counters + net.num_layers, f.n_chain, t);
    if (t.tid == 0) {
        const int before = DTQN_AGENT_ADD(f.counters + kFuseDeparted, (int32_t)1);
        if (before == f.n_role - 1)
            for (int e = 0; e <= kFuseDeparted; ++e) DTQN_AGENT_STORE(f.counters + e, (int32_t)0);
    }
}

__device__ __forceinline__ void fuse_arrive(int32_t* counters, int e, const Thr& t) {
    if (t.tid == 0) DTQN_AGENT_ADD(counters + e, (int32_t)1);
}

inline int fuse_cu_count() { return device_cu_count(); }
inline bool fuse_plan(const DtqnNet* net, const DtqnTd* td, FuseArgs* f) {
    f->n_role = 0;
    if (!net || !td || td->row_split != 4 || net->tiled || net->gate == DTQN_GATE_GRU || net->identity || net->bag_size > 0 || net->img_c > 0 ||
        dtqn_ws_lite(net->tiled, net->d_model, net->head_dim, net->d_real))
        return false;
    if (!td->grad || !td->norm_partial || !td->step_counter || !td->small || !td->xflags || !td->act || !td->grd) return false;
    if (!dtqn_td_wgrad_is_direct(net, td->batch) || waves_for(*net) != kFuseWaves) return false;
    const int NL = net->num_layers;
    if (net->n_wjobs != 1 + 4 * NL + 2 || net->n_wjobs > kFuseMaxJobs || NL + 1 > kFuseMaxEvents) return false;
    const char* e = getenv("DTQN_WGRAD_FUSED");
    if (e == nullptr || atoi(e) == 0) return false;
    DtqnWJob jobs[kFuseMaxJobs];
    if (dtqn_net_wjobs(net, jobs) != DTQN_OK) return false;
    if (net->grd_stride % 32 != 0 || net->go_dq % 32 != 0 || net->go_dhh % 32 != 0 || net->go_dx0 % 32 != 0 ||
        net->go_layer0 % 32 != 0 || net->grd_layer_stride % 32 != 0 || net->lp % 32 != 0)
        return false;
    for (int j = 0; j < net->n_wjobs; ++j)
        if (!jobs[j].x_in_act) return false;
    const int n_chain = td->batch * 4;
    int n_role = ((fuse_cu_count() - n_chain) / 8) * 8;
    const char* r = getenv("DTQN_FUSE_ROLE_WGS");
    if (r != nullptr) n_role = (atoi(r) / 8) * 8;
    const int n_parts = dtqn_td_norm_partials(net);
    if (n_role > n_parts) n_role = (n_parts / 8) * 8;
    if (n_role < 8) return false;
    int tiles = 0;
    for (int k = 0; k < net->n_wjobs; ++k) {
        const int j = net->n_wjobs - 1 - k;
        f->jobs[k] = jobs[j];
        f->dtile0[k] = tiles;
        tiles += direct_tiles_of(jobs[j]);
        const int layer = j == 0 ? 0 : j > 4 * NL ? NL - 1 : (j - 1) / 4;
        f->job_event[k] = (j == 0 || layer == 0) ? NL : NL - 1 - layer;
    }
    f->n_jobs = net->n_wjobs;
    f->n_tiles = tiles;
    f->n_small = small_elems(net);
    f->n_items = tiles + (f->n_small + kDSmallFused - 1) / kDSmallFused;
    f->n_parts = n_parts;
    f->n_chain = n_chain;
    f->grad = td->grad;
    f->norm_partial = td->norm_partial;
    f->step_counter = td->step_counter;
    f->counters = td->xflags + dtqn_td_xch_flags(net, td->batch) - kFuseWords;
    f->n_role = n_role;
    return true;
}

}
```

### include/dtqn_hip.h

```cpp
#ifndef DTQN_HIP_H
#define DTQN_HIP_H

#include <stddef.h>
#include <stdint.h>

#ifdef __cplusplus
extern "C" {
#endif

#define DTQN_ABI_VERSION 21
#define DTQN_MAX_LAYERS 8

#define DTQN_OK 0
#define DTQN_ERR_CONFIG 1
#define DTQN_ERR_ARG 2
#define DTQN_ERR_LAUNCH 3

#define DTQN_GATE_RES 0
#define DTQN_GATE_GRU 1
#define DTQN_POS_LEARNED 0
#define DTQN_POS_SIN 1
#define DTQN_POS_NONE 2

typedef struct DtqnNet {
    int32_t obs_dim;
    int32_t num_actions;
    int32_t embed_per_obs;
    int32_t action_dim;
    int32_t d_model;
    int32_t num_heads;
    int32_t num_layers;
    int32_t ctx_len;
    int32_t gate;
    int32_t identity;
    int32_t pos;
    int32_t discrete;
    int32_t vocab;
    int32_t force_tiled;
    int32_t bag_size;
    int32_t img_c, img_h, img_w;
    float dropout;
    int32_t d_real, heads_real, hd_real;
    int32_t abi_version;
    int32_t lp;
    int32_t ke;
    int32_t kep;
    int32_t ap;
    int32_t head_dim;
    int32_t ffn_chunk;
    int32_t tiled;
    int32_t off_act_emb;
    int32_t off_obs_tab;
    int32_t off_obs_w;
    int32_t off_obs_b;
    int32_t off_pos;
    int32_t off_layer0;
    int32_t layer_stride;
    int32_t lo_ln1_w, lo_ln1_b, lo_ln2_w, lo_ln2_b;
    int32_t lo_in_w, lo_in_b, lo_out_w, lo_out_b;
    int32_t lo_f1_w, lo_f1_b, lo_f2_w, lo_f2_b;
    int32_t off_gate_attn;
    int32_t off_gate_mlp;
    int32_t go_w_r, go_u_r, go_w_z, go_b_z, go_u_z, go_w_g, go_u_g;
    int32_t off_head1_w, off_head1_b, off_head2_w, off_head2_b;
    int32_t off_bag_in_w, off_bag_in_b, off_bag_out_w, off_bag_out_b;
    int32_t off_cw0, off_cw1, off_cw2, off_cw3, off_cw4;
    int32_t off_cb0, off_cb1, off_cb2, off_cb3, off_cb4;
    int32_t img_h1, img_w1, img_h3, img_w3, img_h5, img_w5;
    int32_t img_feat;
    int32_t img_k1;
    int32_t n_trainable;
    int32_t n_theta;
    int32_t act_stride;
    int32_t ao_ein, ao_x0, ao_layer0, act_layer_stride, ao_xf, ao_hh;
    int32_t al_u1, al_qkv, al_lse, al_o, al_m1, al_s1, al_st1, al_u2, al_h, al_mh, al_m2, al_s2, al_st2;
    int32_t al_gate1, al_gate2;
    int32_t ao_bag_ein, ao_bag_e, ao_bag_kv, ao_bag_q, ao_bag_p, ao_bag_o, ao_xcat, bag_ld;
    int32_t grd_stride;
    int32_t go_dx0, go_layer0, grd_layer_stride, go_dhh, go_dq;
    int32_t gl_dqkv, gl_da, gl_dhp, gl_df;
    int32_t gl_gate1, gl_gate2;
    int32_t go_do;
    int32_t go_dcat, go_bag_do, go_bag_dq, go_bag_dkv, go_bag_de;
    int32_t sp_stride;
    int32_t so_ln, so_tab, so_act;
    int32_t sp_parts;
    int32_t n_wjobs;
    int32_t n_wtiles;
} DtqnNet;

typedef struct DtqnWJob {
    int32_t x_in_act;
    int32_t x_off, ldx, K;
    int32_t dy_off, ldy, N;
    int32_t w_off;
    int32_t b_off;
    int32_t tile0;
    int32_t tiles_n, tiles_k;
    int32_t n_layers;
    int32_t x_lstride;
    int32_t dy_lstride;
} DtqnWJob;

int dtqn_net_init(DtqnNet* net);
int dtqn_net_wjobs(const DtqnNet* net, DtqnWJob* jobs);
int dtqn_net_fill_frozen(const DtqnNet* net, float* theta_host);
int dtqn_lds_bytes_forward(const DtqnNet* net, int training);
int dtqn_lds_bytes_backward(const DtqnNet* net);

typedef struct DtqnReplay {
    float* obs;
    uint8_t* actions;
    float* rewards;
    uint8_t* dones;
    int32_t* ep_len;
    uint8_t* obs_u8;
    int32_t num_episodes;
    int32_t max_steps;
    int32_t obs_dim;
    float obs_mask;
} DtqnReplay;

typedef struct DtqnReplayRecord {
    int32_t kind;
    int32_t ep;
    int32_t t;
    int32_t action;
    float reward;
    int32_t done;
    int32_t obs_index;
    int32_t ep_len;
} DtqnReplayRecord;

int dtqn_replay_apply(const DtqnReplay* rp, const DtqnReplayRecord* recs_dev, const float* obs_rows_dev,
                      int n, void* stream);
int dtqn_replay_gather_bag(const DtqnReplay* rp, const int32_t* ep_idx_dev, const int32_t* start_dev, const int32_t* rows_dev,
                           int batch, int bag_size, uint32_t seed, const int32_t* step_counter_dev, float* bag_obs_dev,
                           uint8_t* bag_actions_dev, void* stream);
int dtqn_replay_sample(const DtqnReplay* rp, int n_valid, int exclude, int ctx_len, int batch, uint32_t seed,
                       const int32_t* step_counter_dev, int32_t* ep_idx_dev, int32_t* start_dev, void* stream);
int dtqn_replay_sample_at(const DtqnReplay* rp, int n_valid, int exclude, int ctx_len, int batch, uint32_t seed, int step,
                          const int32_t* step_counter_dev, int32_t* ep_idx_dev, int32_t* start_dev, void* stream);

int dtqn_forward(const DtqnNet* net, const float* theta, const float* obs, const uint8_t* actions,
                 int batch, int n, float* q_out, void* stream);

int dtqn_forward_workspace_floats(const DtqnNet* net, int batch);
int dtqn_forward_tiled(const DtqnNet* net, const float* theta, const float* obs, const uint8_t* actions,
                       int batch, int n, float* q_out, float* workspace, void* stream);

typedef struct DtqnTd {
    float* theta_pol;
    float* theta_tgt;
    float* grad;
    float* adam_m;
    float* adam_v;
    int32_t* ep_idx;
    int32_t* start;
    float* act;
    float* grd;
    float* small;
    float* q3;
    float* gsplit;
    float* norm_partial;
    float* stats_partial;
    float* stats;
    float* stats_ring;
    int32_t* step_counter;
    const DtqnWJob* wjobs;
    float* xch;
    int32_t* xflags;
    float* bag_obs;
    uint8_t* bag_actions;
    const int32_t* xstatus;
    const float* xemb;
    float* wpack_pol;
    float* wpack_tgt;
    int32_t batch;
    int32_t history;
    int32_t n_split;
    int32_t n_norm_blocks;
    int32_t stats_ring_slots;
    int32_t target_update_frequency;
    int32_t sample_in_kernel;
    int32_t sample_n_valid;
    int32_t sample_exclude;
    uint32_t sample_seed;
    uint32_t dropout_seed;
    int32_t row_split;
    int32_t xch_timeout_ms;
    int32_t side_stream;
    float gamma;
    float lr;
    float beta1;
    float beta2;
    float eps;
    float grad_norm_clip;
    float grad_scale;
} DtqnTd;


int dtqn_replay_push(const DtqnReplay* rp, const DtqnReplayRecord* recs_host, const float* obs_host, int n, void* stream);

int dtqn_actor_forward(const DtqnNet* net, const float* theta, const void* ctx_host, void* ctx_dev, int n, float* q_dev,
                       float* q_last_host, float* workspace, int train_mode, uint32_t dropout_seed, uint32_t dropout_step,
                       void* stream);

int dtqn_actor_forward_batch(const DtqnNet* net, const float* theta, const void* ctx_host, void* ctx_dev, int n_envs, int n_max,
                             float* q_dev, float* q_last_host, float* workspace, int train_mode, uint32_t dropout_seed,
                             uint32_t dropout_step, void* stream);
int dtqn_actor_greedy_batch(const DtqnNet* net, const float* theta, const void* ctx_host, void* ctx_dev, int n_envs, int n_max,
                            float* q_dev, float* q_last_host, int32_t* action_host, float* workspace, int train_mode,
                            uint32_t dropout_seed, uint32_t dropout_step, void* stream);
int dtqn_debug_last_actor_live(void);
int dtqn_forward_bag(const DtqnNet* net, const float* theta, const float* obs, const uint8_t* actions, const float* bag_obs,
                     const uint8_t* bag_actions, int batch, int n, float* q_out, float* workspace, int train_mode,
                     uint32_t dropout_seed, uint32_t dropout_step, void* stream);
int dtqn_forward_tiled_strided(const DtqnNet* net, const float* theta, const float* obs, const uint8_t* actions, int batch, int n,
                               int in_rows, float* q_out, float* workspace, void* stream);

int dtqn_td_row_split(const DtqnNet* net, int batch);
int dtqn_td_latency_mode(const DtqnNet* net, int batch);
int dtqn_td_prefers_tiled(const DtqnNet* net, int batch);
int dtqn_net_tiled_twin(const DtqnNet* src, DtqnNet* dst);
int dtqn_td_xch_floats(const DtqnNet* net, int batch);
int dtqn_td_xch_flags(const DtqnNet* net, int batch);

int dtqn_td_forward(const DtqnNet* net, const DtqnReplay* rp, const DtqnTd* td, void* stream);
int dtqn_td_forward_part(const DtqnNet* net, const DtqnReplay* rp, const DtqnTd* td, int pass0, int npasses, int slices, int draw_step,
                         void* stream);
int dtqn_td_fwd_slices4_ok(const DtqnNet* net);
int dtqn_td_backward(const DtqnNet* net, const DtqnReplay* rp, const DtqnTd* td, void* stream);
int dtqn_td_backward_ahead(const DtqnNet* net, const DtqnReplay* rp, const DtqnTd* td, const DtqnTd* td_next, int draw_step_next, void* stream);
int dtqn_td_wgrad(const DtqnNet* net, const DtqnTd* td, void* stream);
int dtqn_td_wgrad_is_direct(const DtqnNet* net, int batch);
int dtqn_td_wgrad_splits(const DtqnNet* net, int batch);
int dtqn_td_wpack_floats(const DtqnNet* net);
int dtqn_td_wpack(const DtqnNet* net, const DtqnTd* td, void* stream);
int dtqn_td_wgrad_is_fused(const DtqnNet* net, const DtqnTd* td);
int dtqn_td_reduce(const DtqnNet* net, const DtqnTd* td, void* stream);
int dtqn_td_norm_partials(const DtqnNet* net);
int dtqn_td_gradnorm(const DtqnNet* net, const DtqnTd* td, void* stream);
int dtqn_td_clip_adam(const DtqnNet* net, const DtqnTd* td, void* stream);
int dtqn_xch_publish(int32_t* own_flag_dev, int32_t gen, void* stream);
int dtqn_td_xreduce(const DtqnNet* net, const DtqnTd* td, const void* peer_grad_ptrs_dev, const void* peer_flag_ptrs_dev, int world,
                    int32_t gen, float* gsum_dev, int32_t* status_dev, int32_t* own_flag_dev, void* stream);
int dtqn_td_update(const DtqnNet* net, const DtqnReplay* rp, const DtqnTd* td, void* stream);
int dtqn_td_update_pipelined(const DtqnNet* net, const DtqnReplay* rp, const DtqnTd* td, const DtqnTd* td_next, int have_target,
                             int draw_step, void* stream);
int dtqn_td_gradients_pipelined(const DtqnNet* net, const DtqnReplay* rp, const DtqnTd* td, const DtqnTd* td_next, int have_target,
                                int draw_step, void* stream);
int dtqn_target_sync(const DtqnNet* net, const float* theta_pol, float* theta_tgt, void* stream);

int dtqn_img_prep_floats(const DtqnNet* net);
long long dtqn_img_act_floats(const DtqnNet* net, int tokens);
long long dtqn_img_wpart_floats(const DtqnNet* net);
int dtqn_img_prep(const DtqnNet* net, const float* theta, float* wprep, void* stream);
int dtqn_img_encode(const DtqnNet* net, const float* theta, const float* wprep, const uint8_t* images_u8, const int32_t* img_index,
                    int tokens, float* act, float* out0, const int32_t* dst0, float* out1, const int32_t* dst1, void* stream);
long long dtqn_img_gact_floats(const DtqnNet* net, int tokens);
int dtqn_img_backward(const DtqnNet* net, const float* theta, const float* wprep, const uint8_t* images_u8, const int32_t* img_index,
                      int tokens, const float* act, const float* dxemb_base, const int32_t* dsrc, float* gact, float* wpart,
                      float* grad_out, void* stream);
int dtqn_img_td_lists(const DtqnNet* net, const DtqnReplay* rp, const DtqnTd* td, int32_t* pol_index, int32_t* pol_dst0, int32_t* pol_dst1,
                      int32_t* pol_dsrc, int32_t* tgt_index, int32_t* tgt_dst0, void* stream);
int dtqn_forward_tiled_pre(const DtqnNet* net, const float* theta, const float* xemb, const uint8_t* actions, int batch, int n,
                           float* q_out, float* workspace, int train_mode, uint32_t dropout_seed, uint32_t dropout_step, void* stream);

long long dtqn_img_actor_stage_bytes(const DtqnNet* net, int n_envs);
long long dtqn_img_actor_workspace_floats(const DtqnNet* net, int n_envs);
int dtqn_img_actor_forward_batch(const DtqnNet* net, const float* theta, float* wprep, int refresh_prep, const void* stage_host,
                                 uint8_t* frame_ring, float* emb_ring, int n_envs, float* q_dev, float* q_last_host, float* workspace,
                                 int train_mode, uint32_t dropout_seed, uint32_t dropout_step, void* stream);
int dtqn_img_actor_greedy_batch(const DtqnNet* net, const float* theta, float* wprep, int refresh_prep, const void* stage_host,
                                uint8_t* frame_ring, float* emb_ring, int n_envs, float* q_dev, float* q_last_host, int32_t* action_host,
                                float* workspace, int train_mode, uint32_t dropout_seed, uint32_t dropout_step, void* stream);
int dtqn_debug_last_img_actor_tokens(void);

long long dtqn_grad_workspace_floats(const DtqnNet* net, int batch, int n);
int dtqn_forward_train(const DtqnNet* net, const float* theta, const float* obs, const uint8_t* actions, const float* bag_obs,
                       const uint8_t* bag_actions, int batch, int n, float* q_out, float* workspace, void* stream);
int dtqn_backward_dq(const DtqnNet* net, const float* theta, const float* obs, const uint8_t* actions, const float* bag_obs,
                     const uint8_t* bag_actions, int batch, int n, const float* dq, float* workspace, float* grad, float* dobs,
                     void* stream);
int dtqn_forward_train_drop(const DtqnNet* net, const float* theta, const float* obs, const uint8_t* actions, const float* bag_obs,
                            const uint8_t* bag_actions, int batch, int n, float* q_out, float* workspace, uint32_t dropout_seed,
                            int32_t dropout_step, void* stream);
int dtqn_backward_dq_drop(const DtqnNet* net, const float* theta, const float* obs, const uint8_t* actions, const float* bag_obs,
                          const uint8_t* bag_actions, int batch, int n, const float* dq, float* workspace, float* grad, float* dobs,
                          uint32_t dropout_seed, int32_t dropout_step, void* stream);
int dtqn_attn_weights(const DtqnNet* net, const float* workspace, int batch, int n, float* alpha_out, float* bag_out, void* stream);

int dtqn_debug_set_profile_buffer(void* dev_buffer);
int dtqn_debug_last_packed_blocks(void);

int dtqn_abi_version(void);
const char* dtqn_build_info(void);

#ifdef __cplusplus
}
#endif
#endif
```

Before: 11680 TD-updates/s.

## Fuse clip-Adam optimizer into direct wgrad kernel via producer/consumer tail blocks

When the direct (non-fused) wgrad path is used on a single device, the separate reduce and clip_adam launches are replaced by one kernel. Extra consumer blocks wait on an arrival counter and then run the clip-norm Adam update, reading gradients and norm partials through coherent stores and loads. This removes kernel launch and inter-kernel gaps on a small per-step workload. In exchange it adds spin-wait synchronisation and write-through stores, and a deadlock risk if consumer blocks become resident before producer blocks. It can be disabled with an environment variable.

```diff
diff --git a/dtqn_amd/_binding.py b/dtqn_amd/_binding.py
--- a/dtqn_amd/_binding.py
+++ b/dtqn_amd/_binding.py
@@ -115,6 +115,7 @@
         "dtqn_td_reduce": [P(DtqnNet), P(DtqnTd), vp],
         "dtqn_td_gradnorm": [P(DtqnNet), P(DtqnTd), vp],
         "dtqn_td_clip_adam": [P(DtqnNet), P(DtqnTd), vp],
+        "dtqn_td_wgrad_adam": [P(DtqnNet), P(DtqnTd), vp],
         "dtqn_img_prep_floats": [P(DtqnNet)],
         "dtqn_img_act_floats": [P(DtqnNet), i32],
         "dtqn_img_gact_floats": [P(DtqnNet), i32],
diff --git a/dtqn_amd/csrc/dtqn_api.cpp b/dtqn_amd/csrc/dtqn_api.cpp
--- a/dtqn_amd/csrc/dtqn_api.cpp
+++ b/dtqn_amd/csrc/dtqn_api.cpp
@@ -88,10 +88,24 @@
     if ((rc = dtqn_td_wgrad(net, td, stream)) != DTQN_OK) return rc;
     return dtqn_td_reduce(net, td, stream);
 }
+static bool adam_tail(const DtqnNet* net, const DtqnTd* td) {
+    if (!net || !td || td->xstatus != nullptr || td->xflags == nullptr) return false;
+    const char* e = getenv("DTQN_ADAM_TAIL");
+    if (e != nullptr && atoi(e) == 0) return false;
+    return dtqn_td_wgrad_is_direct(net, td->batch) && !dtqn_td_wgrad_is_fused(net, td);
+}
 extern "C" int dtqn_td_update_pipelined(const DtqnNet* net, const DtqnReplay* rp, const DtqnTd* td, const DtqnTd* td_next, int have_target,
                                         int draw_step, void* stream) {
-    const int rc = dtqn_td_gradients_pipelined(net, rp, td, td_next, have_target, draw_step, stream);
-    return rc != DTQN_OK ? rc : dtqn_td_clip_adam(net, td, stream);
+    if (!adam_tail(net, td)) {
+        const int rc = dtqn_td_gradients_pipelined(net, rp, td, td_next, have_target, draw_step, stream);
+        return rc != DTQN_OK ? rc : dtqn_td_clip_adam(net, td, stream);
+    }
+    int rc;
+    if (draw_step < 0) return DTQN_ERR_ARG;
+    if ((rc = dtqn_td_forward_part(net, rp, td, 0, 2, 4, draw_step, stream)) != DTQN_OK) return rc;
+    if (!have_target && (rc = dtqn_td_forward_part(net, rp, td, 2, 1, 4, draw_step, stream)) != DTQN_OK) return rc;
+    rc = td_next != nullptr ? dtqn_td_backward_ahead(net, rp, td, td_next, draw_step + 1, stream) : dtqn_td_backward(net, rp, td, stream);
+    return rc != DTQN_OK ? rc : dtqn_td_wgrad_adam(net, td, stream);
 }
 
 namespace dtqn {
diff --git a/dtqn_amd/csrc/dtqn_clip_adam.hpp b/dtqn_amd/csrc/dtqn_clip_adam.hpp
--- /dev/null
+++ b/dtqn_amd/csrc/dtqn_clip_adam.hpp
@@ -0,0 +1,160 @@
+#pragma once
+#include "dtqn_device.hpp"
+
+namespace dtqn {
+
+constexpr int kOptThreads = 256;
+constexpr int kOptVec = 4;
+constexpr int kOptBlockElems = kOptThreads * kOptVec;
+
+__device__ __forceinline__ float block_sum(float v, float* red, int tid) {
+    for (int m = 32; m >= 1; m >>= 1) v += __shfl_xor(v, m);
+    if ((tid & 63) == 0) red[tid >> 6] = v;
+    __syncthreads();
+    float s = 0.f;
+    for (int w = 0; w < kOptThreads / 64; ++w) s += red[w];
+    __syncthreads();
+    return s;
+}
+
+struct AdamArgs {
+    float* theta;
+    float* theta_tgt;
+    const float* grad;
+    float* m;
+    float* v;
+    const float* norm_partial;
+    const float* stats_partial;
+    float* stats;
+    float* stats_ring;
+    int32_t* step_counter;
+    const int32_t* xstatus;
+    int n, n_norm_parts, batch, history, tuf, ring_slots;
+    int n_stat_parts;
+    float lr, beta1, beta2, eps, clip, grad_scale;
+};
+
+template <int G, bool TAIL, typename Wait>
+__device__ __forceinline__ void clip_adam_blocks(const AdamArgs& a, int blk0, int nblk, int wtid, Wait&& wait) {
+    __shared__ float red[G][kOptThreads / 64];
+    __shared__ double pw[G][2];
+    const int grp = G > 1 ? wtid / kOptThreads : 0, tid = wtid - grp * kOptThreads;
+    const int blk = blk0 + grp;
+    const int p0 = (blk * kOptThreads + tid) * kOptVec;
+    const bool mine = blk < nblk && p0 < a.n;
+    const float4 z4 = make_float4(0.f, 0.f, 0.f, 0.f);
+    float4 g4 = z4;
+    if constexpr (!TAIL) g4 = mine ? ld4(a.grad + p0) : z4;
+    float4 m4 = mine ? ld4(a.m + p0) : z4, v4 = mine ? ld4(a.v + p0) : z4, p4 = mine ? ld4(a.theta + p0) : z4;
+    const DtqnRsrc grs = DTQN_XCH_RSRC(a.grad, (size_t)a.n * 4), nrs = DTQN_XCH_RSRC(a.norm_partial, (size_t)a.n_norm_parts * 4);
+    if constexpr (TAIL) {
+        DTQN_SCHED_FENCE();
+        wait();
+        if (mine) g4 = dtqn_xch_load4(grs, p0 * 4);
+    }
+    float part = 0.f;
+    if constexpr (TAIL) {
+        for (int i = tid; i < a.n_norm_parts; i += 2 * kOptThreads) {
+            const bool two = i + kOptThreads < a.n_norm_parts;
+            const float x0 = dtqn_xch_load1(nrs, i * 4), x1 = dtqn_xch_load1(nrs, (two ? i + kOptThreads : i) * 4);
+            part += x0;
+            if (two) part += x1;
+        }
+    } else {
+        for (int i = tid; i < a.n_norm_parts; i += kOptThreads) part += a.norm_partial[i];
+    }
+    const float total = block_sum(part, red[grp], tid);
+    const float norm = sqrtf(total) * a.grad_scale;
+    const int sticky = TAIL ? DTQN_AGENT_LOAD(a.step_counter + 3) : a.step_counter[3];
+    const int why = !isfinite(norm) ? 1 : (a.xstatus != nullptr && *a.xstatus != 0) ? 2 : (sticky != 0) ? 3 : 0;
+    const bool finite = why == 0;
+    const int k = (TAIL ? DTQN_AGENT_LOAD(a.step_counter) : a.step_counter[0]) + 1;
+    if (tid == 0 || tid == 64) {
+        const double beta = tid == 0 ? (double)a.beta1 : (double)a.beta2;
+        double r = 1.0, b = beta;
+        for (unsigned e = (unsigned)k; e != 0u; e >>= 1) {
+            if (e & 1u) r *= b;
+            b *= b;
+        }
+        pw[grp][tid >> 6] = 1.0 - r;
+    }
+    __syncthreads();
+    const float bc1 = (float)pw[grp][0], bc2_sqrt = (float)sqrt(pw[grp][1]);
+    const float coef = fminf(1.0f, a.clip / (norm + 1e-6f)) * a.grad_scale;
+    const float step_size = a.lr / bc1;
+    const bool sync_target = finite && a.tuf > 0 && (k % a.tuf) == 0;
+    if (finite && mine) {
+        const float g[4] = {g4.x * coef, g4.y * coef, g4.z * coef, g4.w * coef};
+        float mm[4] = {m4.x, m4.y, m4.z, m4.w}, vv[4] = {v4.x, v4.y, v4.z, v4.w}, pp[4] = {p4.x, p4.y, p4.z, p4.w};
+#pragma unroll
+        for (int c = 0; c < 4; ++c) {
+            mm[c] = mm[c] + (g[c] - mm[c]) * (1.0f - a.beta1);
+            vv[c] = vv[c] * a.beta2 + (1.0f - a.beta2) * g[c] * g[c];
+            const float denom = sqrtf(vv[c]) / bc2_sqrt + a.eps;
+            pp[c] = pp[c] - step_size * (mm[c] / denom);
+        }
+        st4(a.m + p0, make_float4(mm[0], mm[1], mm[2], mm[3]));
+        st4(a.v + p0, make_float4(vv[0], vv[1], vv[2], vv[3]));
+        const float4 pn = make_float4(pp[0], pp[1], pp[2], pp[3]);
+        st4(a.theta + p0, pn);
+        if (sync_target) st4(a.theta_tgt + p0, pn);
+    }
+    if (nblk - 1 >= blk0 && nblk - 1 < blk0 + G) {
+        const bool last = blk == nblk - 1;
+        float se = 0.f, sq = 0.f, sy = 0.f, mxq = -INFINITY, mnq = INFINITY, mxy = -INFINITY, mny = INFINITY;
+        const int call_prev = !last ? 0 : TAIL ? DTQN_AGENT_LOAD(a.step_counter + 2) : a.step_counter[2];
+        for (int b = tid; b < (last ? a.n_stat_parts : 0); b += kOptThreads) {
+            const float* sp = a.stats_partial + (size_t)b * 8;
+            se += sp[0]; sq += sp[1]; mxq = fmaxf(mxq, sp[2]); mnq = fminf(mnq, sp[3]);
+            sy += sp[4]; mxy = fmaxf(mxy, sp[5]); mny = fminf(mny, sp[6]);
+        }
+        se = block_sum(se, red[grp], tid); sq = block_sum(sq, red[grp], tid); sy = block_sum(sy, red[grp], tid);
+        for (int mk = 32; mk >= 1; mk >>= 1) {
+            mxq = fmaxf(mxq, __shfl_xor(mxq, mk)); mnq = fminf(mnq, __shfl_xor(mnq, mk));
+            mxy = fmaxf(mxy, __shfl_xor(mxy, mk)); mny = fminf(mny, __shfl_xor(mny, mk));
+        }
+        __shared__ float mm4[G][4][kOptThreads / 64];
+        if ((tid & 63) == 0) { mm4[grp][0][tid >> 6] = mxq; mm4[grp][1][tid >> 6] = mnq; mm4[grp][2][tid >> 6] = mxy; mm4[grp][3][tid >> 6] = mny; }
+        __syncthreads();
+        if (last && tid == 0) {
+            for (int w = 1; w < kOptThreads / 64; ++w) {
+                mxq = fmaxf(mxq, mm4[grp][0][w]); mnq = fminf(mnq, mm4[grp][1][w]); mxy = fmaxf(mxy, mm4[grp][2][w]); mny = fminf(mny, mm4[grp][3][w]);
+            }
+            const float cnt = (float)a.batch * (float)a.history;
+            a.stats[0] = se / cnt;
+            a.stats[1] = norm;
+            a.stats[2] = mxq; a.stats[3] = sq / cnt; a.stats[4] = mnq;
+            a.stats[5] = mxy; a.stats[6] = sy / cnt; a.stats[7] = mny;
+            a.stats[8] = fminf(1.0f, a.clip / (norm + 1e-6f));
+            a.stats[9] = (float)k;
+            a.stats[10] = sync_target ? 1.f : 0.f;
+            a.stats[11] = (float)why;
+            if (finite) a.step_counter[1] = k;
+            else a.step_counter[3] = 1;
+            const int call = call_prev + 1;
+            a.step_counter[2] = call;
+            if (a.stats_ring != nullptr) {
+                unsigned long long* slot = reinterpret_cast<unsigned long long*>(a.stats_ring) + (size_t)((call - 1) % a.ring_slots) * 12;
+                const unsigned long long tag = (unsigned long long)__float_as_uint((float)(call & 0x7fffff)) << 32;
+                const float vals[12] = {se / cnt, norm, mxq, sq / cnt, mnq, mxy, sy / cnt, mny, fminf(1.0f, a.clip / (norm + 1e-6f)), (float)k,
+                                        sync_target ? 1.f : 0.f, (float)why};
+                for (int i = 0; i < 12; ++i) DTQN_SYSTEM_STORE(slot + i, tag | (unsigned long long)__float_as_uint(vals[i]));
+            }
+        }
+    }
+}
+
+inline void fill_adam_args(const DtqnNet* net, const DtqnTd* td, int n_norm_parts, AdamArgs* a) {
+    a->theta = td->theta_pol; a->theta_tgt = td->theta_tgt; a->grad = td->grad; a->m = td->adam_m; a->v = td->adam_v;
+    a->norm_partial = td->norm_partial; a->stats_partial = td->stats_partial; a->stats = td->stats;
+    a->step_counter = td->step_counter;
+    a->xstatus = td->xstatus;
+    a->stats_ring = td->stats_ring; a->ring_slots = td->stats_ring_slots > 0 ? td->stats_ring_slots : 1;
+    a->n = net->n_trainable; a->n_norm_parts = n_norm_parts; a->batch = td->batch; a->history = td->history;
+    a->n_stat_parts = td->batch * (td->row_split > 1 ? td->row_split : 1);
+    a->tuf = td->target_update_frequency;
+    a->lr = td->lr; a->beta1 = td->beta1; a->beta2 = td->beta2; a->eps = td->eps; a->clip = td->grad_norm_clip;
+    a->grad_scale = td->grad_scale;
+}
+
+}
diff --git a/dtqn_amd/csrc/dtqn_optim.hip b/dtqn_amd/csrc/dtqn_optim.hip
--- a/dtqn_amd/csrc/dtqn_optim.hip
+++ b/dtqn_amd/csrc/dtqn_optim.hip
@@ -1,12 +1,9 @@
 #include <cstdlib>
 
 #include "dtqn_device.hpp"
+#include "dtqn_clip_adam.hpp"
 
 namespace dtqn {
-
-constexpr int kOptThreads = 256;
-constexpr int kOptVec = 4;
-constexpr int kOptBlockElems = kOptThreads * kOptVec;
 
 struct ReduceArgs {
     DtqnNet net;
@@ -19,16 +16,6 @@
     int batch, n_split;
     int n_parts;
 };
-
-__device__ __forceinline__ float block_sum(float v, float* red, int tid) {
-    for (int m = 32; m >= 1; m >>= 1) v += __shfl_xor(v, m);
-    if ((tid & 63) == 0) red[tid >> 6] = v;
-    __syncthreads();
-    float s = 0.f;
-    for (int w = 0; w < kOptThreads / 64; ++w) s += red[w];
-    __syncthreads();
-    return s;
-}
 
 __global__ __launch_bounds__(kOptThreads) void dtqn_reduce_kernel(ReduceArgs a) {
     __shared__ float red[kOptThreads / 64];
@@ -120,111 +107,8 @@
     if (tid == 0) a.norm_partial[blockIdx.x] = ss;
 }
 
-struct AdamArgs {
-    float* theta;
-    float* theta_tgt;
-    const float* grad;
-    float* m;
-    float* v;
-    const float* norm_partial;
-    const float* stats_partial;
-    float* stats;
-    float* stats_ring;
-    int32_t* step_counter;
-    const int32_t* xstatus;
-    int n, n_norm_parts, batch, history, tuf, ring_slots;
-    int n_stat_parts;
-    float lr, beta1, beta2, eps, clip, grad_scale;
-};
-
 __global__ __launch_bounds__(kOptThreads) void dtqn_clip_adam_kernel(AdamArgs a) {
-    __shared__ float red[kOptThreads / 64];
-    __shared__ double pw[2];
-    const int tid = (int)threadIdx.x;
-    const int p0 = ((int)blockIdx.x * kOptThreads + tid) * kOptVec;
-    const bool mine = p0 < a.n;
-    const float4 z4 = make_float4(0.f, 0.f, 0.f, 0.f);
-    const float4 g4 = mine ? ld4(a.grad + p0) : z4;
-    float4 m4 = mine ? ld4(a.m + p0) : z4, v4 = mine ? ld4(a.v + p0) : z4, p4 = mine ? ld4(a.theta + p0) : z4;
-    float part = 0.f;
-    for (int i = tid; i < a.n_norm_parts; i += kOptThreads) part += a.norm_partial[i];
-    const float total = block_sum(part, red, tid);
-    const float norm = sqrtf(total) * a.grad_scale;
-    const int why = !isfinite(norm) ? 1 : (a.xstatus != nullptr && *a.xstatus != 0) ? 2 : (a.step_counter[3] != 0) ? 3 : 0;
-    const bool finite = why == 0;
-    const int k = a.step_counter[0] + 1;
-    if (tid == 0 || tid == 64) {
-        const double beta = tid == 0 ? (double)a.beta1 : (double)a.beta2;
-        double r = 1.0, b = beta;
-        for (unsigned e = (unsigned)k; e != 0u; e >>= 1) {
-            if (e & 1u) r *= b;
-            b *= b;
-        }
-        pw[tid >> 6] = 1.0 - r;
-    }
-    __syncthreads();
-    const float bc1 = (float)pw[0], bc2_sqrt = (float)sqrt(pw[1]);
-    const float coef = fminf(1.0f, a.clip / (norm + 1e-6f)) * a.grad_scale;
-    const float step_size = a.lr / bc1;
-    const bool sync_target = finite && a.tuf > 0 && (k % a.tuf) == 0;
-    if (finite && mine) {
-        const float g[4] = {g4.x * coef, g4.y * coef, g4.z * coef, g4.w * coef};
-        float mm[4] = {m4.x, m4.y, m4.z, m4.w}, vv[4] = {v4.x, v4.y, v4.z, v4.w}, pp[4] = {p4.x, p4.y, p4.z, p4.w};
-#pragma unroll
-        for (int c = 0; c < 4; ++c) {
-            mm[c] = mm[c] + (g[c] - mm[c]) * (1.0f - a.beta1);
-            vv[c] = vv[c] * a.beta2 + (1.0f - a.beta2) * g[c] * g[c];
-            const float denom = sqrtf(vv[c]) / bc2_sqrt + a.eps;
-            pp[c] = pp[c] - step_size * (mm[c] / denom);
-        }
-        st4(a.m + p0, make_float4(mm[0], mm[1], mm[2], mm[3]));
-        st4(a.v + p0, make_float4(vv[0], vv[1], vv[2], vv[3]));
-        const float4 pn = make_float4(pp[0], pp[1], pp[2], pp[3]);
-        st4(a.theta + p0, pn);
-        if (sync_target) st4(a.theta_tgt + p0, pn);
-    }
-    if (blockIdx.x == gridDim.x - 1) {
-        float se = 0.f, sq = 0.f, sy = 0.f, mxq = -INFINITY, mnq = INFINITY, mxy = -INFINITY, mny = INFINITY;
-        const int call_prev = a.step_counter[2];
-        for (int b = tid; b < a.n_stat_parts; b += kOptThreads) {
-            const float* sp = a.stats_partial + (size_t)b * 8;
-            se += sp[0]; sq += sp[1]; mxq = fmaxf(mxq, sp[2]); mnq = fminf(mnq, sp[3]);
-            sy += sp[4]; mxy = fmaxf(mxy, sp[5]); mny = fminf(mny, sp[6]);
-        }
-        se = block_sum(se, red, tid); sq = block_sum(sq, red, tid); sy = block_sum(sy, red, tid);
-        for (int mk = 32; mk >= 1; mk >>= 1) {
-            mxq = fmaxf(mxq, __shfl_xor(mxq, mk)); mnq = fminf(mnq, __shfl_xor(mnq, mk));
-            mxy = fmaxf(mxy, __shfl_xor(mxy, mk)); mny = fminf(mny, __shfl_xor(mny, mk));
-        }
-        __shared__ float mm4[4][kOptThreads / 64];
-        if ((tid & 63) == 0) { mm4[0][tid >> 6] = mxq; mm4[1][tid >> 6] = mnq; mm4[2][tid >> 6] = mxy; mm4[3][tid >> 6] = mny; }
-        __syncthreads();
-        if (tid == 0) {
-            for (int w = 1; w < kOptThreads / 64; ++w) {
-                mxq = fmaxf(mxq, mm4[0][w]); mnq = fminf(mnq, mm4[1][w]); mxy = fmaxf(mxy, mm4[2][w]); mny = fminf(mny, mm4[3][w]);
-            }
-            const float cnt = (float)a.batch * (float)a.history;
-            a.stats[0] = se / cnt;
-            a.stats[1] = norm;
-            a.stats[2] = mxq; a.stats[3] = sq / cnt; a.stats[4] = mnq;
-            a.stats[5] = mxy; a.stats[6] = sy / cnt; a.stats[7] = mny;
-            a.stats[8] = fminf(1.0f, a.clip / (norm + 1e-6f));
-            a.stats[9] = (float)k;
-            a.stats[10] = sync_target ? 1.f : 0.f;
-            a.stats[11] = (float)why;
-            if (finite) a.step_counter[1] = k;
-            else a.step_counter[3] = 1;
-            const int call = call_prev + 1;
-            a.step_counter[2] = call;
-            if (a.stats_ring != nullptr) {
-                unsigned long long* slot = reinterpret_cast<unsigned long long*>(a.stats_ring) + (size_t)((call - 1) % a.ring_slots) * 12;
-                const unsigned long long tag = (unsigned long long)__float_as_uint((float)(call & 0x7fffff)) << 32;
-                const float vals[12] = {se / cnt, norm, mxq, sq / cnt, mnq, mxy, sy / cnt, mny, fminf(1.0f, a.clip / (norm + 1e-6f)), (float)k,
-                                        sync_target ? 1.f : 0.f, (float)why};
-                for (int i = 0; i < 12; ++i) DTQN_SYSTEM_STORE(slot + i, tag | (unsigned long long)__float_as_uint(vals[i]));
-            }
-        }
-    }
+    clip_adam_blocks<1, false>(a, (int)blockIdx.x, (int)gridDim.x, (int)threadIdx.x, [] {});
 }
 
 struct CopyArgs {
@@ -298,16 +182,7 @@
     if (!net || !td) return DTQN_ERR_ARG;
     if (td->n_norm_blocks != opt_blocks(net->n_trainable)) return DTQN_ERR_ARG;
     AdamArgs a;
-    a.theta = td->theta_pol; a.theta_tgt = td->theta_tgt; a.grad = td->grad; a.m = td->adam_m; a.v = td->adam_v;
-    a.norm_partial = td->norm_partial; a.stats_partial = td->stats_partial; a.stats = td->stats;
-    a.step_counter = td->step_counter;
-    a.xstatus = td->xstatus;
-    a.stats_ring = td->stats_ring; a.ring_slots = td->stats_ring_slots > 0 ? td->stats_ring_slots : 1;
-    a.n = net->n_trainable; a.n_norm_parts = dtqn_td_norm_partials(net); a.batch = td->batch; a.history = td->history;
-    a.n_stat_parts = td->batch * (td->row_split > 1 ? td->row_split : 1);
-    a.tuf = td->target_update_frequency;
-    a.lr = td->lr; a.beta1 = td->beta1; a.beta2 = td->beta2; a.eps = td->eps; a.clip = td->grad_norm_clip;
-    a.grad_scale = td->grad_scale;
+    fill_adam_args(net, td, dtqn_td_norm_partials(net), &a);
     (void)hipGetLastError();
     hipLaunchKernelGGL(dtqn_clip_adam_kernel, dim3(td->n_norm_blocks + 1), dim3(kOptThreads), 0, (hipStream_t)stream, a);
     return hipGetLastError() == hipSuccess ? DTQN_OK : DTQN_ERR_LAUNCH;
diff --git a/dtqn_amd/csrc/dtqn_wgrad.hip b/dtqn_amd/csrc/dtqn_wgrad.hip
--- a/dtqn_amd/csrc/dtqn_wgrad.hip
+++ b/dtqn_amd/csrc/dtqn_wgrad.hip
@@ -1,6 +1,7 @@
 #include <mutex>
 #include "dtqn_device.hpp"
 #include "dtqn_wgrad_direct.hpp"
+#include "dtqn_clip_adam.hpp"
 
 namespace dtqn {
 
@@ -365,6 +366,60 @@
     direct_norm_partial<kDirectWaves>(ss, red, a.norm_partial, b, t);
 }
 
+constexpr int kTailGroups = kDirectThreads / kOptThreads;
+constexpr int kTailArrived = kFuseWords - 2, kTailDeparted = kFuseWords - 1;
+static_assert(kTailArrived > kFuseDeparted, "the tail's counters are not the fused backward's");
+static_assert(kDirectThreads % kOptThreads == 0, "whole optimizer blocks per consumer workgroup");
+struct TailArgs {
+    AdamArgs opt;
+    int32_t* counters;
+    int n_prod;
+    int n_opt;
+    int n_cons;
+};
+
+__global__ __launch_bounds__(kDirectThreads) void dtqn_wgrad_adam_kernel(WgradDirectArgs a, TailArgs o) {
+    const Thr t = make_thr();
+    const int tid = t.tid, b = (int)blockIdx.x;
+    if (b >= o.n_prod) {
+        clip_adam_blocks<kTailGroups, true>(o.opt, (b - o.n_prod) * kTailGroups, o.n_opt, tid, [&] {
+            if (tid == 0) {
+                while (DTQN_AGENT_LOAD(o.counters + kTailArrived) < o.n_prod) DTQN_SPIN_PAUSE_LONG();
+                const int before = DTQN_AGENT_ADD(o.counters + kTailDeparted, (int32_t)1);
+                if (before == o.n_cons - 1) {
+                    DTQN_AGENT_STORE(o.counters + kTailArrived, (int32_t)0);
+                    DTQN_AGENT_STORE(o.counters + kTailDeparted, (int32_t)0);
+                }
+            }
+            __syncthreads();
+        });
+        return;
+    }
+    const DtqnNet& net = a.net;
+    float* red = reinterpret_cast<float*>(dtqn_smem);
+    float* slabs = red + kDirectWaves;
+    float ss = 0.f;
+    const int tile_blocks = a.slots * 8;
+    if (b == 0 && tid == 0) DTQN_AGENT_STORE(a.step_counter, a.step_counter[1]);
+    if (b == 0)
+        for (int i = o.n_prod + tid; i < a.n_parts; i += kDirectThreads) DTQN_AGENT_STORE(a.norm_partial + i, 0.f);
+    const int tile = b >= tile_blocks ? a.n_tiles : !a.xcd_map ? b : b / 8 < a.xcd_ntiles[b % 8] ? a.xcd_tile0[b % 8] + b / 8 : a.n_tiles;
+    const DirectCtx ctx{a.act, a.grd, a.small, a.grad, a.batch, a.row_split, a.n_small};
+    if (b >= tile_blocks) {
+        ss = a.small_per == 2 * kDSmall ? direct_small<false, 2 * kDSmall, kDirectWaves, true>(net, ctx, b - tile_blocks, slabs, t)
+                                        : direct_small<false, kDSmall, kDirectWaves, true>(net, ctx, b - tile_blocks, slabs, t);
+    } else if (tile < a.n_tiles) {
+        int j = 0;
+        for (int k = 1; k < a.n_jobs; ++k)
+            if (a.dtile0[k] <= tile) j = k;
+        ss = direct_tile<false, kDirectWaves, true>(net, ctx, a.jobs[j], tile - a.dtile0[j], slabs, t);
+    }
+    direct_norm_partial<kDirectWaves, true>(ss, red, a.norm_partial, b, t);
+    DTQN_WAIT_VMEM();
+    __syncthreads();
+    if (tid == 0) DTQN_AGENT_ADD(o.counters + kTailArrived, (int32_t)1);
+}
+
 static int direct_tiles(const DtqnNet* net, const DtqnWJob* jobs, int* dtile0) {
     int tiles = 0;
     for (int j = 0; j < net->n_wjobs; ++j) {
@@ -444,7 +499,7 @@
     return opt > dir ? opt : dir;
 }
 
-static int wgrad_direct(const DtqnNet* net, const DtqnTd* td, hipStream_t stream) {
+static int wgrad_direct(const DtqnNet* net, const DtqnTd* td, hipStream_t stream, bool adam_tail = false) {
     WgradDirectArgs a;
     a.net = *net;
     if (dtqn_net_wjobs(net, a.jobs) != DTQN_OK) return DTQN_ERR_CONFIG;
@@ -464,7 +519,17 @@
     const int grid = plan.grid;
     const size_t lds = kDirectLdsFloats * sizeof(float);
     (void)hipGetLastError();
-    hipLaunchKernelGGL(dtqn_wgrad_direct_kernel, dim3(grid), dim3(kDirectThreads), lds, stream, a);
+    if (adam_tail) {
+        TailArgs o;
+        fill_adam_args(net, td, a.n_parts, &o.opt);
+        o.counters = td->xflags + dtqn_td_xch_flags(net, td->batch) - kFuseWords;
+        o.n_prod = grid;
+        o.n_opt = td->n_norm_blocks + 1;
+        o.n_cons = (o.n_opt + kTailGroups - 1) / kTailGroups;
+        hipLaunchKernelGGL(dtqn_wgrad_adam_kernel, dim3(grid + o.n_cons), dim3(kDirectThreads), lds, stream, a, o);
+    } else {
+        hipLaunchKernelGGL(dtqn_wgrad_direct_kernel, dim3(grid), dim3(kDirectThreads), lds, stream, a);
+    }
     return hipGetLastError() == hipSuccess ? DTQN_OK : DTQN_ERR_LAUNCH;
 }
 
@@ -487,6 +552,14 @@
         (void)hipGetLastError();
     }
     return l.state == 1 ? &l : nullptr;
+}
+
+extern "C" int dtqn_td_wgrad_adam(const DtqnNet* net, const DtqnTd* td, void* stream) {
+    if (!net || !td || td->batch < 1 || td->n_split < 1) return DTQN_ERR_ARG;
+    if (net->n_wjobs > kMaxWJobs) return DTQN_ERR_CONFIG;
+    if (td->n_norm_blocks != (net->n_trainable + kOptBlockElems - 1) / kOptBlockElems || !td->xflags || td->xstatus != nullptr) return DTQN_ERR_ARG;
+    if (dtqn_td_wgrad_is_fused(net, td) || !dtqn_td_wgrad_is_direct(net, td->batch)) return DTQN_ERR_CONFIG;
+    return wgrad_direct(net, td, (hipStream_t)stream, true);
 }
 
 extern "C" int dtqn_td_wgrad(const DtqnNet* net, const DtqnTd* td, void* stream) {
diff --git a/dtqn_amd/csrc/dtqn_wgrad_direct.hpp b/dtqn_amd/csrc/dtqn_wgrad_direct.hpp
--- a/dtqn_amd/csrc/dtqn_wgrad_direct.hpp
+++ b/dtqn_amd/csrc/dtqn_wgrad_direct.hpp
@@ -34,7 +34,18 @@
     else return base[idx];
 }
 
-template <bool SC1, int WV>
+template <bool WT>
+__device__ __forceinline__ void direct_st4(float* base, const DtqnRsrc& rs, size_t idx, float4 v) {
+    if constexpr (WT) dtqn_xch_store4(rs, (int)(idx * 4), v);
+    else st4(base + idx, v);
+}
+template <bool WT>
+__device__ __forceinline__ void direct_st1(float* base, const DtqnRsrc& rs, size_t idx, float v) {
+    if constexpr (WT) dtqn_xch_store1(rs, (int)(idx * 4), v);
+    else base[idx] = v;
+}
+
+template <bool SC1, int WV, bool WT = false>
 __device__ __forceinline__ float direct_tile(const DtqnNet& net, const DirectCtx& a, const DtqnWJob& job, int local, float* slabs, const Thr& t) {
     const int LP = net.lp, tid = t.tid;
     float ss = 0.f;
@@ -47,6 +58,7 @@
     const size_t xstride = job.x_in_act ? (size_t)net.act_stride : (size_t)net.grd_stride;
     const size_t ystride = (size_t)net.grd_stride;
     const DtqnRsrc grs = DTQN_XCH_RSRC(a.grd, (size_t)a.batch * net.grd_stride * 4);
+    const DtqnRsrc ors = DTQN_XCH_RSRC(a.grad, (size_t)net.n_trainable * 4);
     const int ycol = nbase + t.i, xcol = kbase + 2 * t.i;
     const bool yok = ycol < job.ldy, xok = xcol < job.ldx;
     f32x4 acc[2] = {zero4(), zero4()};
@@ -145,14 +157,14 @@
                 const float4 x = ld4(slabs + (size_t)w * (kDTN + 1) * SLD + nl * SLD + k4);
                 v.x += x.x; v.y += x.y; v.z += x.z; v.w += x.w;
             }
-            float* op = a.grad + job.w_off + (size_t)n * job.K + k;
+            const size_t op = (size_t)job.w_off + (size_t)n * job.K + k;
             if (k + 3 < job.K && (job.K & 3) == 0) {
-                st4(op, v);
+                direct_st4<WT>(a.grad, ors, op, v);
                 ss = (v.x * v.x + v.y * v.y) + (v.z * v.z + v.w * v.w);
             } else {
                 const float vv[4] = {v.x, v.y, v.z, v.w};
                 for (int c = 0; c < 4; ++c)
-                    if (k + c < job.K) { op[c] = vv[c]; ss += vv[c] * vv[c]; }
+                    if (k + c < job.K) { direct_st1<WT>(a.grad, ors, op + c, vv[c]); ss += vv[c] * vv[c]; }
             }
         }
     } else if (tid >= 256 && tid < 256 + kDTN && job.b_off >= 0 && bk == 0) {
@@ -161,14 +173,14 @@
             float v = 0.f;
 #pragma unroll
             for (int w = 0; w < WV; ++w) v += slabs[(size_t)w * (kDTN + 1) * SLD + kDTN * SLD + nl];
-            a.grad[job.b_off + n] = v;
+            direct_st1<WT>(a.grad, ors, (size_t)(job.b_off + n), v);
             ss = v * v;
         }
     }
     return ss;
 }
 
-template <bool SC1, int PER, int WV>
+template <bool SC1, int PER, int WV, bool WT = false>
 __device__ __forceinline__ float direct_small(const DtqnNet& net, const DirectCtx& a, int sb, float* slabs, const Thr& t) {
     constexpr int HN = PER / 64;
     static_assert(HN <= WV, "one finishing wave per 64 elements");
@@ -178,6 +190,7 @@
     const int n_act = net.action_dim > 0 ? net.num_actions * net.action_dim : 0;
     const DtqnRsrc grs = DTQN_XCH_RSRC(a.grd, (size_t)a.batch * net.grd_stride * 4);
     const DtqnRsrc srs = DTQN_XCH_RSRC(a.small, (size_t)a.batch * a.row_split * net.sp_parts * net.sp_stride * 4);
+    const DtqnRsrc ors = DTQN_XCH_RSRC(a.grad, (size_t)net.n_trainable * 4);
     float ss = 0.f;
     int dst[HN];
 #pragma unroll
@@ -221,14 +234,14 @@
             float tot = 0.f;
 #pragma unroll
             for (int w = 0; w < WV; ++w) tot += slabs[(t.wave * WV + w) * 64 + t.lane];
-            a.grad[d] = tot;
+            direct_st1<WT>(a.grad, ors, (size_t)d, tot);
             ss = tot * tot;
         }
     }
     return ss;
 }
 
-template <int WV>
+template <int WV, bool WT = false>
 __device__ __forceinline__ void direct_norm_partial(float ss, float* red, float* norm_partial, int slot, const Thr& t) {
     ss = wave_sum(ss);
     __syncthreads();
@@ -237,7 +250,8 @@
     if (t.tid == 0) {
         float tot = 0.f;
         for (int w = 0; w < WV; ++w) tot += red[w];
-        norm_partial[slot] = tot;
+        if constexpr (WT) DTQN_AGENT_STORE(norm_partial + slot, tot);
+        else norm_partial[slot] = tot;
     }
 }
 
diff --git a/include/dtqn_hip.h b/include/dtqn_hip.h
--- a/include/dtqn_hip.h
+++ b/include/dtqn_hip.h
@@ -242,6 +242,7 @@
 int dtqn_td_norm_partials(const DtqnNet* net);
 int dtqn_td_gradnorm(const DtqnNet* net, const DtqnTd* td, void* stream);
 int dtqn_td_clip_adam(const DtqnNet* net, const DtqnTd* td, void* stream);
+int dtqn_td_wgrad_adam(const DtqnNet* net, const DtqnTd* td, void* stream);
 int dtqn_xch_publish(int32_t* own_flag_dev, int32_t gen, void* stream);
 int dtqn_td_xreduce(const DtqnNet* net, const DtqnTd* td, const void* peer_grad_ptrs_dev, const void* peer_flag_ptrs_dev, int world,
                     int32_t gen, float* gsum_dev, int32_t* status_dev, int32_t* own_flag_dev, void* stream);
```

Result: slower. 10870 TD-updates/s (-7.0%).
